# hfeeki/stellard

Hardware: AMD Instinct MI355X
Metric: Ed25519 tx verifies/sec (higher is better)
Workload: dtype u32

## Files before the change

### stellard_amd/build.py

```python
import os
import shutil
import subprocess
import sys

ROOT = os.path.dirname(os.path.dirname(os.path.abspath(__file__)))
CSRC = os.path.join(ROOT, "stellard_amd", "csrc")
HIPCC = shutil.which("hipcc") or "/opt/rocm/bin/hipcc"
ARCH = os.environ.get("PYTORCH_ROCM_ARCH", "gfx950")

PRODUCT_SRCS = ["stl_kernels.hip", "stl_keyset.hip", "stl_api.cpp", "stl_batcher.cpp"]
PRODUCT_DEPS = PRODUCT_SRCS + ["stl_kernels.h", "stl_verify_core.h", "stl_fe25519.h", "stl_ge25519.h",
                               "stl_sc25519.h", "stl_sha512.h", "stl_base_table.h", "stl_lattice.h", "stl_txblob.h", "stl_sign.h",
                               "stl_comb.h", "stl_keyset.h",
                               os.path.join("..", "..", "include", "stl.h")]


def source_digest():
    import hashlib
    h = hashlib.sha256()
    for d in PRODUCT_DEPS:
        with open(os.path.join(CSRC, d), "rb") as f:
            h.update(os.path.basename(d).encode() + b"\0" + f.read())
    return h.hexdigest()


def _stale(out, deps):
    if not os.path.exists(out):
        return True
    t = os.path.getmtime(out)
    return any(os.path.getmtime(d) > t for d in deps)


def _run(cmd, cwd=ROOT):
    print("+", " ".join(cmd), flush=True)
    subprocess.run(cmd, cwd=cwd, check=True)


HOST_DEPS = ["stl_kernels.h", "stl_keyset.h", os.path.join("..", "..", "include", "stl.h")]
OBJ_DIR = os.path.join(ROOT, "build", "obj")


def build_product(force=False, extra_flags=(), variant="variant"):
    out = os.path.join(ROOT, "stellard_amd", "libstl.so")
    deps = [os.path.join(CSRC, d) for d in PRODUCT_DEPS]
    if extra_flags:
        vout = os.path.join(ROOT, "build", "ab", variant + ".so")
        os.makedirs(os.path.dirname(vout), exist_ok=True)
        _run([HIPCC, f"--offload-arch={ARCH}", "-O3", "-std=c++17", "-fPIC", "-shared", *extra_flags,
              "-o", vout] + [os.path.join(CSRC, s) for s in PRODUCT_SRCS])
        return vout
    os.makedirs(OBJ_DIR, exist_ok=True)
    objs = []
    for src in PRODUCT_SRCS:
        obj = os.path.join(OBJ_DIR, src + ".o")
        if src.endswith(".hip"):
            sdeps = [d for d in deps if not d.endswith((".hip", ".cpp")) or d.endswith(src)]
        else:
            sdeps = [os.path.join(CSRC, d) for d in [src] + HOST_DEPS]
        if force or _stale(obj, sdeps):
            _run([HIPCC, f"--offload-arch={ARCH}", "-O3", "-std=c++17", "-fPIC", "-c", "-o", obj,
                  os.path.join(CSRC, src)])
        objs.append(obj)
    if force or _stale(out, objs):
        _run([HIPCC, f"--offload-arch={ARCH}", "-fPIC", "-shared", "-o", out] + objs)
    return out


def build_hostemu(force=False):
    out = os.path.join(ROOT, "tests", "native", "libhostemu.so")
    src = os.path.join(ROOT, "tests", "native", "hostemu.cpp")
    deps = [src] + [os.path.join(CSRC, d) for d in PRODUCT_DEPS]
    if force or _stale(out, deps):
        _run([HIPCC, "-O2", "-std=c++17", "-fPIC", "-shared", "-o", out, src])
    return out


def build_hostemu_keyset(force=False):
    out = os.path.join(ROOT, "tests", "native", "libhostemu_keyset.so")
    src = os.path.join(ROOT, "tests", "native", "hostemu_keyset.cpp")
    deps = [src] + [os.path.join(CSRC, d) for d in PRODUCT_DEPS]
    if force or _stale(out, deps):
        _run([HIPCC, "-O2", "-std=c++17", "-fPIC", "-shared", "-o", out, src])
    return out


def build_oracle():
    oracle = os.path.join(ROOT, "oracle")
    targets = ["build/liboracle.so"]
    if os.path.exists("/opt/conda/include/sodium.h"):
        targets.append("_ref/libsodium_ref.so")
    _run(["make", "-s", "-C", oracle] + targets)


def main(argv=None):
    argv = sys.argv[1:] if argv is None else argv
    force = "--force" in argv
    if "--product-only" in argv:
        build_product(force=force)
        return
    from concurrent.futures import ThreadPoolExecutor
    with ThreadPoolExecutor(max_workers=3) as ex:
        jobs = [ex.submit(build_product, force), ex.submit(build_hostemu, force),
                ex.submit(build_hostemu_keyset, force)]
        for j in jobs:
            j.result()
    build_oracle()


if __name__ == "__main__":
    main()
```

### stellard_amd/csrc/stl_api.cpp

```cpp
#include <dlfcn.h>
#include <hip/hip_runtime.h>
#include <rccl/rccl.h>

#include <algorithm>
#include <array>
#include <atomic>
#include <chrono>
#include <cstddef>
#include <cstdio>
#include <cstdlib>
#include <cstring>
#include <map>
#include <memory>
#include <mutex>
#include <set>
#include <thread>
#include <vector>

#include "../../include/stl.h"
#include "stl_kernels.h"
#include "stl_keyset.h"

namespace {

std::atomic<long long> g_fault_after{-1};

bool fault_now() {
  long long v = g_fault_after.load(std::memory_order_relaxed);
  while (v >= 0) {
    if (g_fault_after.compare_exchange_weak(v, v - 1, std::memory_order_relaxed)) return v == 0;
  }
  return false;
}

#define STL_TRY(expr)                        \
  do {                                       \
    if (fault_now()) return STL_EHIP;        \
    hipError_t e_ = (expr);                  \
    if (e_ != hipSuccess) return STL_EHIP;   \
  } while (0)

#define STL_RCCL_TRY(expr)                   \
  do {                                       \
    if (fault_now()) return STL_ERCCL;       \
    ncclResult_t r_ = (expr);                \
    if (r_ != ncclSuccess) return STL_ERCCL; \
  } while (0)

#define STL_RC(expr)        \
  do {                      \
    int rc_ = (expr);       \
    if (rc_) return rc_;    \
  } while (0)

struct Rccl {
  std::once_flag once;
  bool ok = false;
  decltype(&ncclGetUniqueId) GetUniqueId = nullptr;
  decltype(&ncclCommInitRank) CommInitRank = nullptr;
  decltype(&ncclCommInitAll) CommInitAll = nullptr;
  decltype(&ncclCommDestroy) CommDestroy = nullptr;
  decltype(&ncclGather) Gather = nullptr;
  decltype(&ncclAllGather) AllGather = nullptr;
  decltype(&ncclSend) Send = nullptr;
  decltype(&ncclRecv) Recv = nullptr;
  decltype(&ncclGroupStart) GroupStart = nullptr;
  decltype(&ncclGroupEnd) GroupEnd = nullptr;
  decltype(&ncclCommCount) CommCount = nullptr;
  decltype(&ncclCommUserRank) CommUserRank = nullptr;
  decltype(&ncclCommInitRankConfig) CommInitRankConfig = nullptr;
  decltype(&ncclCommGetAsyncError) CommGetAsyncError = nullptr;
  decltype(&ncclCommAbort) CommAbort = nullptr;
  bool nonblocking() const { return CommInitRankConfig && CommGetAsyncError && CommAbort; }

  template <typename F>
  static bool sym(void* h, const char* name, F& f) {
    f = reinterpret_cast<F>(dlsym(h, name));
    return f != nullptr;
  }
  bool load() {
    std::call_once(once, [this] {
      void* h = dlopen("librccl.so.1", RTLD_NOW | RTLD_GLOBAL);
      if (!h) h = dlopen("/opt/rocm/lib/librccl.so.1", RTLD_NOW | RTLD_GLOBAL);
      if (!h) return;
      ok = sym(h, "ncclGetUniqueId", GetUniqueId) && sym(h, "ncclCommInitRank", CommInitRank) &&
           sym(h, "ncclCommInitAll", CommInitAll) && sym(h, "ncclCommDestroy", CommDestroy) &&
           sym(h, "ncclGather", Gather) && sym(h, "ncclAllGather", AllGather) && sym(h, "ncclSend", Send) &&
           sym(h, "ncclRecv", Recv) && sym(h, "ncclGroupStart", GroupStart) && sym(h, "ncclGroupEnd", GroupEnd) &&
           sym(h, "ncclCommCount", CommCount) && sym(h, "ncclCommUserRank", CommUserRank);
      (void)(sym(h, "ncclCommInitRankConfig", CommInitRankConfig) &&
             sym(h, "ncclCommGetAsyncError", CommGetAsyncError) && sym(h, "ncclCommAbort", CommAbort));
    });
    return ok;
  }
};
Rccl g_rccl;

std::atomic<int> g_rccl_timeout_ms{120000};

int rccl_settle(ncclComm_t comm, ncclResult_t r) {
  if (r == ncclSuccess) return STL_OK;
  if (r != ncclInProgress || !comm || !g_rccl.CommGetAsyncError) return STL_ERCCL;
  const auto end = std::chrono::steady_clock::now() + std::chrono::milliseconds(g_rccl_timeout_ms.load());
  ncclResult_t st = ncclInProgress;
  while (g_rccl.CommGetAsyncError(comm, &st) == ncclSuccess && st == ncclInProgress) {
    if (std::chrono::steady_clock::now() > end) return STL_ERCCL;
    std::this_thread::sleep_for(std::chrono::microseconds(200));
  }
  return st == ncclSuccess ? STL_OK : STL_ERCCL;
}

struct DevBuf {
  void* p = nullptr;
  size_t cap = 0;
  int ensure(size_t bytes) {
    if (bytes <= cap) return STL_OK;
    if (p) (void)hipFree(p);
    p = nullptr;
    cap = 0;
    if (fault_now() || hipMalloc(&p, bytes) != hipSuccess) {
      p = nullptr;
      return STL_ENOMEM;
    }
    cap = bytes;
    return STL_OK;
  }
  void release() {
    if (p) (void)hipFree(p);
    p = nullptr;
    cap = 0;
  }
};

struct PhaseTimer {
  std::mutex mu;
  std::vector<hipEvent_t> pool;
  std::vector<std::array<hipEvent_t, 5>> done;
  uint64_t ns[4] = {0, 0, 0, 0};
  uint64_t chunks = 0;
  hipEvent_t take() {
    std::lock_guard<std::mutex> lk(mu);
    if (!pool.empty()) {
      hipEvent_t e = pool.back();
      pool.pop_back();
      return e;
    }
    hipEvent_t e = nullptr;
    if (hipEventCreate(&e) != hipSuccess) e = nullptr;
    return e;
  }
  void give(hipEvent_t e) {
    if (!e) return;
    std::lock_guard<std::mutex> lk(mu);
    pool.push_back(e);
  }
  void collect() {
    std::lock_guard<std::mutex> lk(mu);
    std::vector<std::array<hipEvent_t, 5>> pending;
    for (auto& c : done) {
      if (hipEventQuery(c[4]) == hipErrorNotReady) {
        pending.push_back(c);
        continue;
      }
      uint64_t t[4];
      bool ok = true;
      for (int i = 0; i < 4 && ok; ++i) {
        float ms = 0.f;
        ok = hipEventElapsedTime(&ms, c[i], c[i + 1]) == hipSuccess;
        t[i] = (uint64_t)((double)ms * 1e6);
      }
      if (ok) {
        for (int i = 0; i < 4; ++i) ns[i] += t[i];
        ++chunks;
      }
      for (hipEvent_t e : c) pool.push_back(e);
    }
    done.swap(pending);
  }
  void reset() {
    collect();
    std::lock_guard<std::mutex> lk(mu);
    for (auto& v : ns) v = 0;
    chunks = 0;
  }
  void release() {
    std::lock_guard<std::mutex> lk(mu);
    for (auto& c : done)
      for (hipEvent_t e : c) pool.push_back(e);
    done.clear();
    for (hipEvent_t e : pool) (void)hipEventDestroy(e);
    pool.clear();
  }
};

std::atomic<bool> g_phase_timing{false};

thread_local std::array<hipEvent_t, 5> t_marks;
thread_local bool t_marks_ok = false;

void phase_mark(void* ctx, hipStream_t s, int i) {
  auto* t = static_cast<PhaseTimer*>(ctx);
  if (i == 0) {
    for (hipEvent_t& m : t_marks) {
      if (m) (void)hipEventDestroy(m);
      m = nullptr;
    }
    t_marks_ok = true;
  }
  hipEvent_t e = t->take();
  if (!e || hipEventRecord(e, s) != hipSuccess) {
    t->give(e);
    t_marks[i] = nullptr;
    t_marks_ok = false;
  } else {
    t_marks[i] = e;
  }
  if (i == 4) {
    if (t_marks_ok) {
      std::lock_guard<std::mutex> lk(t->mu);
      t->done.push_back(t_marks);
    } else {
      for (hipEvent_t m : t_marks) t->give(m);
    }
    t_marks.fill(nullptr);
    t_marks_ok = false;
  }
}

std::atomic<int> g_tune_fused{1};
std::atomic<int> g_tune_queue{1};
std::atomic<int> g_tune_streams{2};
std::atomic<int> g_tune_sub_log2{0};
std::atomic<int> g_tune_byte_shards{0};
std::atomic<int> g_tune_quad{3};
std::atomic<int> g_tune_long_hash{8};
std::atomic<int> g_tune_shared_keys{1};
std::atomic<int> g_tune_wide_min{0};
std::atomic<int> g_tune_r_ahead{1};
std::atomic<int> g_tune_first_chunk{0};

std::atomic<uint64_t> g_shard_quantum{65536};

uint32_t pair_max_lanes(uint32_t grid);
uint32_t chunk_for(uint32_t grid, size_t n) {
  const int t = g_tune_sub_log2.load();
  if (t) return 1u << t;
  const size_t pm = pair_max_lanes(grid);
  if (n <= 2 * pm) return (uint32_t)std::min<size_t>(std::max<size_t>(n, 64), stl::kPreChunk);
  if (n <= 3 * pm) return (uint32_t)(2 * pm);
  const size_t nc = std::max<size_t>(2, (n + ((size_t)1 << 17)) >> 18);
  size_t sub = ((n + nc - 1) / nc + 63) / 64 * 64;
  sub = std::max<size_t>(sub, pair_max_lanes(grid) + 64);
  return (uint32_t)std::min<size_t>(sub, stl::kPreChunk);
}

struct StreamCtx;
struct CtxSpares {
  std::mutex mu;
  std::vector<std::unique_ptr<StreamCtx>> list;
};
std::atomic<int>& max_caller_streams();
struct StreamCtx {
  std::mutex mu;
  int ordinal = -1;
  bool pool = false;
  uint64_t last_use = 0;
  hipEvent_t done = nullptr;
  std::weak_ptr<CtxSpares> spares;
  DevBuf ws;
  DevBuf queue;
  hipEvent_t fork = nullptr;
  hipEvent_t join[stl::kMaxVerifyStreams] = {};
  hipEvent_t keys = nullptr;
  hipEvent_t parsed[2] = {};
  DevBuf rdec;
  hipEvent_t rready = nullptr;
  uint32_t* auto_flag = nullptr;
  uint32_t* auto_flag_dev = nullptr;
  DevBuf scratch;
  void release() {
    if (auto_flag) (void)hipHostFree(auto_flag);
    auto_flag = auto_flag_dev = nullptr;
    scratch.release();
    ws.release();
    queue.release();
    for (hipEvent_t& e : join) {
      if (e) (void)hipEventDestroy(e);
      e = nullptr;
    }
    if (fork) (void)hipEventDestroy(fork);
    fork = nullptr;
    if (keys) (void)hipEventDestroy(keys);
    keys = nullptr;
    for (hipEvent_t& e : parsed) {
      if (e) (void)hipEventDestroy(e);
      e = nullptr;
    }
    rdec.release();
    if (rready) (void)hipEventDestroy(rready);
    rready = nullptr;
    if (done) (void)hipEventDestroy(done);
    done = nullptr;
  }
  bool holds_memory() const {
    return auto_flag || scratch.p || ws.p || queue.p || fork || keys || parsed[0] || parsed[1] || rdec.p || rready ||
           done;
  }
  void adopt(StreamCtx& o) {
    std::swap(ws, o.ws);
    std::swap(queue, o.queue);
    std::swap(scratch, o.scratch);
    std::swap(fork, o.fork);
    std::swap(keys, o.keys);
    std::swap(parsed[0], o.parsed[0]);
    std::swap(parsed[1], o.parsed[1]);
    std::swap(rdec, o.rdec);
    std::swap(rready, o.rready);
    for (uint32_t j = 0; j < stl::kMaxVerifyStreams; ++j) std::swap(join[j], o.join[j]);
    std::swap(auto_flag, o.auto_flag);
    std::swap(auto_flag_dev, o.auto_flag_dev);
    std::swap(done, o.done);
  }
  ~StreamCtx() {
    if (!holds_memory() || ordinal < 0) return;
    if (done) {
      if (std::shared_ptr<CtxSpares> sp = spares.lock()) {
        auto z = std::make_unique<StreamCtx>();
        z->ordinal = ordinal;
        z->adopt(*this);
        std::unique_ptr<StreamCtx> over;
        {
          std::lock_guard<std::mutex> lk(sp->mu);
          sp->list.push_back(std::move(z));
          if (sp->list.size() > (size_t)max_caller_streams().load()) {
            over = std::move(sp->list.front());
            sp->list.erase(sp->list.begin());
          }
        }
        return;
      }
    }
    int prev = -1;
    (void)hipGetDevice(&prev);
    if (hipSetDevice(ordinal) == hipSuccess) (void)hipDeviceSynchronize();
    release();
    if (prev >= 0) (void)hipSetDevice(prev);
  }
};

std::unique_ptr<StreamCtx> take_spare(CtxSpares& sp) {
  std::lock_guard<std::mutex> lk(sp.mu);
  if (sp.list.empty()) return nullptr;
  size_t pick = 0;
  for (size_t i = 0; i < sp.list.size(); ++i)
    if (sp.list[i]->done && hipEventQuery(sp.list[i]->done) == hipSuccess) {
      pick = i;
      break;
    }
  std::unique_ptr<StreamCtx> z = std::move(sp.list[pick]);
  sp.list.erase(sp.list.begin() + (long)pick);
  return z;
}

struct Device {
  int ordinal = 0;
  int cus = 0;
  uint32_t grid = 0;
  hipStream_t stream = nullptr;
  hipStream_t stream2 = nullptr;
  hipStream_t copy = nullptr;
  std::atomic<hipStream_t> stream3{nullptr};
  ncclComm_t comm = nullptr;
  std::mutex mu;
  DevBuf sig, msg, pk, bitmap, pre, off, len, ctr, ctr2, txid, status, wide, gather;
  DevBuf counters;
  std::map<hipStream_t, std::shared_ptr<StreamCtx>> stream_ws;
  std::shared_ptr<CtxSpares> spares = std::make_shared<CtxSpares>();
  uint64_t ws_tick = 0;
  std::mutex ws_mu;
  void* stage = nullptr;
  size_t stage_cap = 0;
  PhaseTimer timer;
  stl::PhaseClock clock{phase_mark, &timer};
};

const stl::PhaseClock* phase_clock(Device& d) { return g_phase_timing.load() ? &d.clock : nullptr; }

std::mutex g_mu;
std::vector<std::unique_ptr<Device>> g_devs;
bool g_init = false;
int g_shards_per_device = 1;
bool g_comm_gather = false;
std::atomic<stl_verify_fn> g_fallback_verify{nullptr};

std::mutex g_pcomm_mu;
ncclComm_t g_pcomm = nullptr;
int g_pcomm_ranks = 0;
hipEvent_t g_gather_start = nullptr;
hipStream_t g_gather_stream = nullptr;

void pcomm_abort_locked() {
  if (g_pcomm && g_rccl.ok) (void)(g_rccl.CommAbort ? g_rccl.CommAbort(g_pcomm) : g_rccl.CommDestroy(g_pcomm));
  g_pcomm = nullptr;
  g_pcomm_ranks = 0;
}

void mark_gather_start(hipStream_t s) {
  if (!g_gather_start && hipEventCreateWithFlags(&g_gather_start, hipEventDisableTiming) != hipSuccess) {
    g_gather_start = nullptr;
    g_gather_stream = nullptr;
    return;
  }
  g_gather_stream = hipEventRecord(g_gather_start, s) == hipSuccess ? s : nullptr;
}

unsigned long long* dev_counters(Device& d) { return static_cast<unsigned long long*>(d.counters.p); }

std::atomic<uint64_t> g_st_batches{0}, g_st_sigs{0}, g_st_errors{0}, g_st_host_ns{0}, g_st_gather_ns{0},
    g_st_auto_dedup{0};
bool g_trace = false;

uint64_t now_ns() {
  return (uint64_t)std::chrono::duration_cast<std::chrono::nanoseconds>(
             std::chrono::steady_clock::now().time_since_epoch())
      .count();
}

struct CallSpan {
  const char* name;
  size_t n;
  uint64_t t0 = now_ns();
  int finish(int rc, uint64_t gather_ns = 0) {
    const uint64_t dt = now_ns() - t0;
    g_st_batches++;
    g_st_sigs += n;
    g_st_host_ns += dt;
    g_st_gather_ns += gather_ns;
    if (rc < 0) g_st_errors++;
    if (g_trace)
      std::fprintf(stderr, "{\"stl_trace\": \"%s\", \"n\": %zu, \"rc\": %d, \"ms\": %.3f, \"gather_ms\": %.3f}\n", name, n,
                   rc, dt * 1e-6, gather_ns * 1e-6);
    return rc;
  }
};

struct DeviceGuard {
  int prev = -1;
  DeviceGuard() {
    if (hipGetDevice(&prev) != hipSuccess) prev = -1;
  }
  ~DeviceGuard() {
    if (prev >= 0) (void)hipSetDevice(prev);
  }
};

int current_device_index() {
  int ord = -1;
  if (hipGetDevice(&ord) != hipSuccess) return -1;
  for (size_t i = 0; i < g_devs.size(); ++i)
    if (g_devs[i]->ordinal == ord) return (int)i;
  return -1;
}

int setup_device(Device& d) {
  STL_TRY(hipSetDevice(d.ordinal));
  hipDeviceProp_t prop;
  STL_TRY(hipGetDeviceProperties(&prop, d.ordinal));
  if (std::strncmp(prop.gcnArchName, "gfx950", 6) != 0) return STL_ENODEV;
  d.cus = prop.multiProcessorCount;
  int per_cu = 0;
  STL_TRY(hipOccupancyMaxActiveBlocksPerMultiprocessor(&per_cu, stl::kernel_verify_msg32(), stl::kBlock, 0));
  if (per_cu < 1) per_cu = 1;
  d.grid = (uint32_t)(d.cus * per_cu);
  g_shard_quantum.store((uint64_t)d.grid * stl::kBlock / 2);
  STL_TRY(hipStreamCreateWithFlags(&d.stream, hipStreamNonBlocking));
  STL_TRY(hipStreamCreateWithFlags(&d.stream2, hipStreamNonBlocking));
  STL_TRY(hipStreamCreateWithFlags(&d.copy, hipStreamNonBlocking));
  STL_RC(d.counters.ensure(64));
  STL_TRY(hipMemsetAsync(d.counters.p, 0, 64, d.stream));
  STL_RC(d.wide.ensure(stl::kWideTableBytes));
  STL_TRY(stl::launch_wide_table(static_cast<uint4*>(d.wide.p), d.stream));
  STL_TRY(hipStreamSynchronize(d.stream));
  return STL_OK;
}

void release_device(Device& d) {
  (void)hipSetDevice(d.ordinal);
  const hipStream_t s3 = d.stream3.load();
  for (hipStream_t s : {d.stream, d.stream2, s3, d.copy})
    if (s) (void)hipStreamSynchronize(s);
  (void)hipDeviceSynchronize();
  if (d.comm && g_rccl.ok) (void)g_rccl.CommDestroy(d.comm);
  d.comm = nullptr;
  for (DevBuf* b : {&d.sig, &d.msg, &d.pk, &d.bitmap, &d.pre, &d.off, &d.len, &d.ctr, &d.ctr2, &d.txid, &d.status,
                    &d.wide, &d.gather, &d.counters})
    b->release();
  {
    std::lock_guard<std::mutex> lk(d.ws_mu);
    for (auto& kv : d.stream_ws) {
      std::lock_guard<std::mutex> cl(kv.second->mu);
      kv.second->release();
    }
    d.stream_ws.clear();
    if (std::shared_ptr<CtxSpares> sp = std::move(d.spares)) {
      std::lock_guard<std::mutex> sl(sp->mu);
      for (auto& z : sp->list) z->release();
      sp->list.clear();
    }
  }
  if (d.stage) (void)hipHostFree(d.stage);
  d.stage = nullptr;
  d.stage_cap = 0;
  d.timer.release();
  for (hipStream_t s : {d.stream, d.stream2, s3, d.copy})
    if (s) (void)hipStreamDestroy(s);
  d.stream = d.stream2 = d.copy = nullptr;
  d.stream3.store(nullptr);
}

int ensure_init() {
  {
    std::lock_guard<std::mutex> lk(g_mu);
    if (g_init) return STL_OK;
  }
  return stl_init(nullptr);
}

constexpr int kDefaultCallerStreams = 8;
std::atomic<int> g_max_caller_streams{kDefaultCallerStreams};
std::atomic<int>& max_caller_streams() { return g_max_caller_streams; }

bool is_pool_stream(const Device& d, hipStream_t s) {
  return s && (s == d.stream || s == d.stream2 || s == d.copy || s == d.stream3.load());
}

struct CtxUse {
  std::shared_ptr<StreamCtx> c;
  hipStream_t s = nullptr;
  ~CtxUse() {
    if (!c || c->pool || !c->done) return;
    std::lock_guard<std::mutex> lk(c->mu);
    (void)hipEventRecord(c->done, s);
  }
};

std::shared_ptr<StreamCtx> stream_ctx(Device& d, hipStream_t s) {
  std::vector<std::shared_ptr<StreamCtx>> evicted;
  std::shared_ptr<StreamCtx> out;
  {
    std::lock_guard<std::mutex> lk(d.ws_mu);
    auto& slot = d.stream_ws[s];
    if (!slot) {
      slot = std::make_shared<StreamCtx>();
      slot->ordinal = d.ordinal;
      slot->pool = is_pool_stream(d, s);
      if (!slot->pool) {
        std::vector<std::pair<uint64_t, hipStream_t>> callers;
        for (auto& kv : d.stream_ws)
          if (!kv.second->pool && kv.first != s) callers.emplace_back(kv.second->last_use, kv.first);
        std::sort(callers.begin(), callers.end());
        const size_t keep = (size_t)std::max(0, g_max_caller_streams.load() - 1);
        for (size_t i = 0; i + keep < callers.size(); ++i) {
          auto it = d.stream_ws.find(callers[i].second);
          evicted.push_back(std::move(it->second));
          d.stream_ws.erase(it);
        }
      }
      if (!slot->pool && d.spares) {
        slot->spares = d.spares;
        StreamCtx* src = nullptr;
        for (auto& e : evicted)
          if (!src && e.use_count() == 1 && e->done) src = e.get();
        std::unique_ptr<StreamCtx> z;
        if (!src && (z = take_spare(*d.spares))) src = z.get();
        if (src) {
          slot->adopt(*src);
          if (slot->done && hipStreamWaitEvent(s, slot->done, 0) != hipSuccess) (void)hipEventSynchronize(slot->done);
        }
        if (!slot->done && hipEventCreateWithFlags(&slot->done, hipEventDisableTiming) != hipSuccess)
          slot->done = nullptr;
      }
    }
    out = d.stream_ws[s];
    out->last_use = ++d.ws_tick;
  }
  if (out->pool) return out;
  auto use = std::make_shared<CtxUse>();
  use->c = out;
  use->s = s;
  return std::shared_ptr<StreamCtx>(use, use->c.get());
}

int caller_contexts(Device& d) {
  std::lock_guard<std::mutex> lk(d.ws_mu);
  int k = 0;
  for (auto& kv : d.stream_ws) k += kv.second->pool ? 0 : 1;
  return k;
}

uint32_t verify_grid_for(const Device& d, size_t n) {
  const size_t tiles = (n + stl::kBlock - 1) / stl::kBlock;
  return (uint32_t)std::max<size_t>(1, std::min<size_t>(2 * tiles, d.grid));
}

uint32_t pair_max_lanes(uint32_t grid) { return grid * stl::kBlock / 4; }
uint32_t pair_max(const Device& d) { return pair_max_lanes(d.grid); }
uint32_t quad_max(const Device& d) { return (g_tune_quad.load() & 1) ? d.grid * stl::kBlock / 16 : 0u; }
uint32_t duo_max(const Device& d) { return (g_tune_quad.load() & 2) ? d.grid * stl::kBlock / 8 : 0u; }

unsigned long long* dev_counters(Device& d);
const stl::PhaseClock* phase_clock(Device& d);

hipStream_t key_stream_for(const Device& d, const hipStream_t* used, uint32_t S) {
  for (hipStream_t c : {d.stream, d.stream2}) {
    bool taken = c == nullptr;
    for (uint32_t j = 0; j < S; ++j) taken = taken || used[j] == c;
    if (!taken) return c;
  }
  return nullptr;
}

int run_verify(Device& d, hipStream_t s, const uint8_t* sig, const uint8_t* msg_or_k, const uint8_t* pk, size_t n,
               uint64_t* words, uint32_t mode, bool pre_k, int streams, bool concurrent = false) {
  const bool dedup = (mode & stl::kModeDedupKeys) != 0;
  stl::VerifyExec x;
  x.grid = verify_grid_for(d, n);
  x.ws_grid = d.grid;
  x.pair_max = pair_max(d);
  x.quad_max = quad_max(d);
  x.duo_max = duo_max(d);
  x.wide = static_cast<const uint4*>(d.wide.p);
  x.counters = dev_counters(d);
  x.clock = phase_clock(d);
  x.fused_prep = g_tune_fused.load();
  x.main_queue = g_tune_queue.load() != 0;
  x.concurrent = concurrent;
  x.sub = chunk_for(d.grid, n);
  x.first = (uint32_t)g_tune_first_chunk.load();
  uint32_t S = (uint32_t)std::max(1, std::min<int>(streams, (int)stl::kMaxVerifyStreams));
  if (x.clock || n <= x.sub || x.sub <= x.pair_max) S = 1;
  S = (uint32_t)std::min<size_t>(S, (n + x.sub - 1) / x.sub);
  hipStream_t pool[stl::kMaxVerifyStreams] = {s};
  uint32_t np = 1;
  if (S > 1) {
    if (S > 3 && !d.stream3.load()) {
      std::lock_guard<std::mutex> lk(d.ws_mu);
      if (!d.stream3.load()) {
        hipStream_t s3 = nullptr;
        STL_TRY(hipStreamCreateWithFlags(&s3, hipStreamNonBlocking));
        d.stream3.store(s3);
      }
    }
    for (hipStream_t p : {d.stream2, d.stream, d.stream3.load()})
      if (np < S && p && p != s) pool[np++] = p;
  }
  S = np;
  x.nstreams = S;
  std::shared_ptr<StreamCtx> hold[stl::kMaxVerifyStreams];
  StreamCtx* ctx[stl::kMaxVerifyStreams];
  for (uint32_t j = 0; j < S; ++j) {
    hold[j] = stream_ctx(d, pool[j]);
    ctx[j] = hold[j].get();
  }
  StreamCtx* order[stl::kMaxVerifyStreams];
  std::copy(ctx, ctx + S, order);
  std::sort(order, order + S);
  std::vector<std::unique_lock<std::mutex>> locks;
  for (uint32_t j = 0; j < S; ++j) locks.emplace_back(order[j]->mu);
  StreamCtx& c = *ctx[0];
  for (uint32_t j = 0; j < S; ++j) {
    STL_RC(ctx[j]->ws.ensure(stl::verify_ws_bytes(d.grid, dedup)));
    x.ws[j] = static_cast<uint4*>(ctx[j]->ws.p);
    x.streams[j] = pool[j];
    if (j > 0) {
      if (!c.join[j]) STL_TRY(hipEventCreateWithFlags(&c.join[j], hipEventDisableTiming));
      x.join[j] = c.join[j];
    }
  }
  if (S > 1 && !c.fork) STL_TRY(hipEventCreateWithFlags(&c.fork, hipEventDisableTiming));
  x.fork = c.fork;
  x.wide_min = (uint32_t)g_tune_wide_min.load();
  if (S > 1 && dedup && g_tune_shared_keys.load()) {
    if (!c.keys) STL_TRY(hipEventCreateWithFlags(&c.keys, hipEventDisableTiming));
    x.key_ready = c.keys;
    x.key_stream = key_stream_for(d, pool, S);
  }
  if (fault_now() || stl::launch_verify(sig, msg_or_k, pk, (uint32_t)n, words, mode, pre_k, x) != hipSuccess) {
    for (uint32_t j = 1; j < S; ++j) (void)hipStreamSynchronize(pool[j]);
    if (x.key_stream) (void)hipStreamSynchronize(x.key_stream);
    return STL_EHIP;
  }
  return STL_OK;
}

int ctx_queue(StreamCtx& c, size_t n, uint32_t** qws, bool blob = false) {
  STL_RC(c.queue.ensure(blob ? stl::blob_queue_bytes(n) : stl::hash_queue_bytes(n)));
  *qws = static_cast<uint32_t*>(c.queue.p);
  return STL_OK;
}

uint32_t hash_grid(const Device& d) { return (uint32_t)d.cus * 8u; }

uint32_t hash_long_min(const Device& d, size_t n) {
  return n <= 2 * (size_t)pair_max(d) ? (uint32_t)g_tune_long_hash.load() : 0u;
}

uint32_t grid_for(const Device& d, size_t n) {
  const size_t tiles = (n + stl::kBlock - 1) / stl::kBlock;
  return (uint32_t)std::max<size_t>(1, std::min<size_t>(tiles, d.grid));
}

void shard(size_t n, int r, int g, size_t* lo, size_t* hi) {
  const size_t words = (n + 63) / 64;
  const size_t per = (words + g - 1) / g;
  *lo = std::min(n, (size_t)r * per * 64);
  *hi = std::min(n, (size_t)(r + 1) * per * 64);
}


void shard_bytes_bounds(const uint32_t* len, size_t n, int g, std::vector<size_t>& bound) {
  bound.assign(g + 1, n);
  bound[0] = 0;
  uint64_t total = 0;
  for (size_t i = 0; i < n; ++i) total += len[i];
  const uint64_t q = g_shard_quantum.load();
  uint64_t acc = 0;
  size_t i = 0;
  for (int r = 1; r < g; ++r) {
    const uint64_t target = (uint64_t)((__uint128_t)total * (unsigned)r / (unsigned)g);
    while (i < n && acc < target) acc += len[i++];
    size_t b = std::min(n, (i + 63) / 64 * 64);
    if (q >= 64 && q % 64 == 0 && n > q) {
      auto prefix = [&](size_t row) {
        uint64_t p = acc;
        if (row >= i)
          for (size_t k = i; k < row; ++k) p += len[k];
        else
          for (size_t k = row; k < i; ++k) p -= len[k];
        return p;
      };
      const size_t down = b / q * q, up = down + q;
      const size_t c = (b - down <= up - b || up > n) ? down : up;
      const uint64_t pc = prefix(c);
      const uint64_t dev = pc > target ? pc - target : target - pc;
      if (c > 0 && c < n && (__uint128_t)dev * (unsigned)g * 40u <= (__uint128_t)total) b = c;
    }
    bound[r] = std::max(bound[r - 1], b);
  }
}

#ifndef STL_PIPE_CHUNK_LOG2
#define STL_PIPE_CHUNK_LOG2 16
#endif
constexpr size_t kPipeChunk = (size_t)1 << STL_PIPE_CHUNK_LOG2;

enum class Mode { kSig, kPre, kBlob };

struct Batch {
  Mode mode;
  const uint8_t *sig, *msg32, *pk, *bytes;
  const uint64_t* off;
  const uint32_t* len;
  uint8_t *bitmap, *status, *txid;
  uint32_t policy, kind;
  bool auto_dedup;
};

const uint8_t* row_key(const Batch& b, size_t i) {
  if (b.mode != Mode::kBlob) return b.pk + 32 * i;
  const uint8_t* p = b.bytes + b.off[i];
  const size_t len = b.len[i], lim = len < 34 ? 0 : std::min<size_t>(len - 34, 256);
  for (size_t j = 0; j + 1 <= lim; ++j)
    if (p[j] == 0x73 && p[j + 1] == 0x20) return p + j + 2;
  return nullptr;
}

bool keys_repeat(const Batch& b, size_t lo, size_t hi) {
  constexpr size_t kSample = 1024, kSlots = 2048;
  const size_t n = hi - lo;
  if (n < 4 * 64) return false;
  const size_t s = std::min(n, kSample);
  uint64_t table[kSlots] = {};
  size_t dups = 0;
  for (size_t k = 0; k < s; ++k) {
    const uint8_t* key = row_key(b, lo + k * n / s);
    if (!key) continue;
    uint64_t a, c;
    std::memcpy(&a, key, 8);
    std::memcpy(&c, key + 24, 8);
    uint64_t f = (a ^ (c * 0x9E3779B97F4A7C15ull)) | 1u;
    size_t h = (size_t)((f * 0xD6E8FEB86659FD93ull) >> 52) & (kSlots - 1);
    while (table[h] && table[h] != f) h = (h + 1) & (kSlots - 1);
    if (table[h] == f) ++dups;
    table[h] = f;
  }
  return 5 * dups >= s;
}

uint32_t chunk_policy(const Batch& b, size_t lo, size_t hi) {
  if (!b.auto_dedup || !keys_repeat(b, lo, hi)) return b.policy;
  g_st_auto_dedup++;
  return b.policy | stl::kModeDedupKeys;
}

struct Shard {
  Device* d = nullptr;
  size_t lo = 0, hi = 0;
  std::vector<uint64_t> roff, row_end;
  std::vector<hipEvent_t> ev;
  int rc = STL_OK;
  ~Shard() {
    for (hipEvent_t e : ev) (void)hipEventDestroy(e);
  }
  int join(hipStream_t from, hipStream_t to) {
    hipEvent_t e;
    STL_TRY(hipEventCreateWithFlags(&e, hipEventDisableTiming));
    ev.push_back(e);
    STL_TRY(hipEventRecord(e, from));
    STL_TRY(hipStreamWaitEvent(to, e, 0));
    return STL_OK;
  }
};

void rebase(const uint64_t* off, const uint32_t* len, size_t lo, size_t hi, std::vector<uint64_t>& roff,
            std::vector<uint64_t>& row_end, uint64_t* base_out, uint64_t* bytes_out) {
  const size_t n = hi - lo;
  uint64_t base = off[lo], end = 0;
  for (size_t i = lo; i < hi; ++i) base = std::min(base, off[i]);
  roff.resize(n);
  row_end.resize(n);
  for (size_t i = 0; i < n; ++i) {
    roff[i] = off[lo + i] - base;
    row_end[i] = roff[i] + len[lo + i];
    end = std::max(end, row_end[i]);
  }
  *base_out = base;
  *bytes_out = end;
}

int copy_rows(Shard& s, uint8_t* dst, const uint8_t* src, size_t c0, size_t c1, uint64_t* watermark) {
  uint64_t need = *watermark;
  for (size_t i = c0; i < c1; ++i) need = std::max(need, s.row_end[i]);
  if (need > *watermark)
    STL_TRY(hipMemcpyAsync(dst + *watermark, src + *watermark, need - *watermark, hipMemcpyHostToDevice, s.d->copy));
  *watermark = need;
  return STL_OK;
}

int enqueue_shard(const Batch& b, Shard& s, size_t words_alloc) {
  Device& d = *s.d;
  const size_t lo = s.lo, n = s.hi - s.lo;
  STL_TRY(hipSetDevice(d.ordinal));
  STL_RC(d.bitmap.ensure(std::max<size_t>(words_alloc, 1) * 8));
  if (n == 0) return STL_OK;
  STL_RC(d.sig.ensure(n * 64));
  STL_RC(d.msg.ensure(n * 32));
  STL_RC(d.pk.ensure(n * 32));
  uint64_t base = 0, bytes = 0, mark = 0;
  uint8_t* dsig = static_cast<uint8_t*>(d.sig.p);
  uint8_t* dmsg = static_cast<uint8_t*>(d.msg.p);
  uint8_t* dpk = static_cast<uint8_t*>(d.pk.p);
  uint8_t* dpre = nullptr;
  uint64_t* doff = nullptr;
  uint32_t* dlen = nullptr;
  if (b.mode != Mode::kSig) {
    rebase(b.off, b.len, lo, s.hi, s.roff, s.row_end, &base, &bytes);
    STL_RC(d.pre.ensure(bytes + 16));
    STL_RC(d.off.ensure(n * 8));
    STL_RC(d.len.ensure(n * 4));
    const size_t qn = std::min(n, kPipeChunk);
    const size_t qbytes = b.mode == Mode::kBlob ? stl::blob_queue_bytes(qn) : stl::hash_queue_bytes(qn);
    STL_RC(d.ctr.ensure(qbytes));
    if (b.mode == Mode::kBlob) {
      STL_RC(d.status.ensure(n));
      if (b.txid) STL_RC(d.txid.ensure(n * 32));
    }
    dpre = static_cast<uint8_t*>(d.pre.p);
    doff = static_cast<uint64_t*>(d.off.p);
    dlen = static_cast<uint32_t*>(d.len.p);
    STL_TRY(hipMemcpyAsync(doff, s.roff.data(), n * 8, hipMemcpyHostToDevice, d.copy));
    STL_TRY(hipMemcpyAsync(dlen, b.len + lo, n * 4, hipMemcpyHostToDevice, d.copy));
  }
  uint8_t* dtxid = (b.mode == Mode::kBlob && b.txid) ? static_cast<uint8_t*>(d.txid.p) : nullptr;
  uint8_t* dstatus = b.mode == Mode::kBlob ? static_cast<uint8_t*>(d.status.p) : nullptr;
  const bool two = g_tune_streams.load() > 1 && n > kPipeChunk && !phase_clock(d);
  if (b.auto_dedup && n > kPipeChunk / 2)
    for (hipStream_t ks : {d.stream, d.stream2}) {
      const std::shared_ptr<StreamCtx> c = stream_ctx(d, ks);
      std::lock_guard<std::mutex> lk(c->mu);
      STL_RC(c->ws.ensure(stl::verify_ws_bytes(d.grid, true)));
    }
  if (two && b.mode != Mode::kSig) {
    const size_t qn = std::min(n, kPipeChunk);
    STL_RC(d.ctr2.ensure(b.mode == Mode::kBlob ? stl::blob_queue_bytes(qn) : stl::hash_queue_bytes(qn)));
  }
  for (size_t c0 = 0; c0 < n; c0 += kPipeChunk) {
    const size_t c1 = std::min(n, c0 + kPipeChunk), cn = c1 - c0;
    const bool odd = two && ((c0 / kPipeChunk) & 1);
    hipStream_t ks = odd ? d.stream2 : d.stream;
    uint32_t* kctr = static_cast<uint32_t*>((odd ? d.ctr2 : d.ctr).p);
    if (b.mode != Mode::kBlob) {
      STL_TRY(hipMemcpyAsync(dsig + 64 * c0, b.sig + 64 * (lo + c0), cn * 64, hipMemcpyHostToDevice, d.copy));
      STL_TRY(hipMemcpyAsync(dpk + 32 * c0, b.pk + 32 * (lo + c0), cn * 32, hipMemcpyHostToDevice, d.copy));
    }
    if (b.mode == Mode::kSig)
      STL_TRY(hipMemcpyAsync(dmsg + 32 * c0, b.msg32 + 32 * (lo + c0), cn * 32, hipMemcpyHostToDevice, d.copy));
    else
      STL_RC(copy_rows(s, dpre, b.bytes + base, c0, c1, &mark));
    STL_RC(s.join(d.copy, ks));
    if (b.mode == Mode::kPre)
      STL_TRY(stl::launch_tx_hash(dpre, doff + c0, dlen + c0, (uint32_t)cn, dmsg + 32 * c0, kctr, hash_grid(d), ks,
                                  hash_long_min(d, n)));
    else if (b.mode == Mode::kBlob)
      STL_TRY(stl::launch_tx_blob(dpre, doff + c0, dlen + c0, (uint32_t)cn, dmsg + 32 * c0, dsig + 64 * c0,
                                  dpk + 32 * c0, dtxid ? dtxid + 32 * c0 : nullptr, dstatus + c0, kctr,
                                  hash_grid(d), ks, b.kind));
    STL_RC(run_verify(d, ks, dsig + 64 * c0, dmsg + 32 * c0, dpk + 32 * c0, cn,
                      static_cast<uint64_t*>(d.bitmap.p) + c0 / 64, chunk_policy(b, lo + c0, lo + c1), false, 1,
                      two));
  }
  if (two) STL_RC(s.join(d.stream2, d.stream));
  if (dstatus && b.status) STL_TRY(hipMemcpyAsync(b.status + lo, dstatus, n, hipMemcpyDeviceToHost, d.stream));
  if (dtxid) STL_TRY(hipMemcpyAsync(b.txid + 32 * lo, dtxid, n * 32, hipMemcpyDeviceToHost, d.stream));
  return STL_OK;
}

int drain(Device& d) {
  (void)hipSetDevice(d.ordinal);
  const hipError_t a = hipStreamSynchronize(d.copy);
  const hipError_t b = hipStreamSynchronize(d.stream);
  const hipError_t c = hipStreamSynchronize(d.stream2);
  const hipStream_t s3 = d.stream3.load();
  const hipError_t e = s3 ? hipStreamSynchronize(s3) : hipSuccess;
  return (a == hipSuccess && b == hipSuccess && c == hipSuccess && e == hipSuccess) ? STL_OK : STL_EHIP;
}

int finish_direct(const Batch& b, Shard& s, std::vector<uint8_t>& host_words) {
  const size_t n = s.hi - s.lo;
  if (n == 0) return STL_OK;
  host_words.resize((n + 63) / 64 * 8);
  STL_TRY(hipMemcpyAsync(host_words.data(), s.d->bitmap.p, host_words.size(), hipMemcpyDeviceToHost, s.d->stream));
  STL_TRY(hipStreamSynchronize(s.d->stream));
  std::memcpy(b.bitmap + s.lo / 8, host_words.data(), (n + 7) / 8);
  return STL_OK;
}

int run_shard_direct(const Batch& b, Shard& s) {
  std::lock_guard<std::mutex> lk(s.d->mu);
  int rc = enqueue_shard(b, s, (s.hi - s.lo + 63) / 64);
  std::vector<uint8_t> host_words;
  if (rc == STL_OK) rc = finish_direct(b, s, host_words);
  const int drc = drain(*s.d);
  return rc ? rc : drc;
}

int gather_to_host(const Batch& b, std::vector<Shard>& sh, size_t n, size_t per, bool equal) {
  const int g = (int)sh.size();
  Device& root = *sh[0].d;
  const size_t words = (n + 63) / 64;
  STL_TRY(hipSetDevice(root.ordinal));
  STL_RC(root.gather.ensure(std::max(words, per * (size_t)g) * 8));
  uint64_t* rbuf = static_cast<uint64_t*>(root.gather.p);
  STL_RCCL_TRY(g_rccl.GroupStart());
  int rc = STL_OK;
  for (int r = 0; r < g; ++r) {
    Device& d = *sh[r].d;
    const uint64_t* sbuf = static_cast<const uint64_t*>(d.bitmap.p);
    if (equal) {
      if (g_rccl.Gather(sbuf, rbuf, per, ncclUint64, 0, d.comm, d.stream) != ncclSuccess) rc = STL_ERCCL;
    } else {
      const size_t w = (sh[r].hi - sh[r].lo + 63) / 64;
      if (w == 0 || r == 0) continue;
      const bool sent = g_rccl.Send(sbuf, w, ncclUint64, 0, d.comm, d.stream) == ncclSuccess;
      const bool recv = g_rccl.Recv(rbuf + sh[r].lo / 64, w, ncclUint64, r, root.comm, root.stream) == ncclSuccess;
      if (!sent || !recv) rc = STL_ERCCL;
    }
  }
  if (g_rccl.GroupEnd() != ncclSuccess && rc == STL_OK) rc = STL_ERCCL;
  if (rc) return rc;
  STL_TRY(hipSetDevice(root.ordinal));
  if (!equal && sh[0].hi > sh[0].lo)
    STL_TRY(hipMemcpyAsync(rbuf, root.bitmap.p, (sh[0].hi - sh[0].lo + 63) / 64 * 8, hipMemcpyDeviceToDevice,
                           root.stream));
  std::vector<uint8_t> host_words(words * 8);
  STL_TRY(hipMemcpyAsync(host_words.data(), rbuf, words * 8, hipMemcpyDeviceToHost, root.stream));
  STL_TRY(hipStreamSynchronize(root.stream));
  std::memcpy(b.bitmap, host_words.data(), (n + 7) / 8);
  return STL_OK;
}

int check_flags(uint32_t flags) {
  return (flags & ~(STL_POLICY_MASK | STL_REQUIRE_S_LT_L | STL_FULL_LENGTH | STL_DEDUP_KEYS | STL_ONE_LANE |
                    STL_NO_AUTO_DEDUP | STL_DEBUG_RAW_PREDICATE))
             ? STL_EINVAL
             : STL_OK;
}

bool auto_dedup(uint32_t flags) {
  return (flags & (STL_DEDUP_KEYS | STL_NO_AUTO_DEDUP | STL_FULL_LENGTH)) == 0;
}

constexpr size_t kSmallBatch = 4096;

int run_small(const Batch& b, size_t n) {
  Device& d = *g_devs[0];
  std::lock_guard<std::mutex> lk(d.mu);
  STL_TRY(hipSetDevice(d.ordinal));
  const size_t bytes = n * 128, words = (n + 63) / 64;
  if (d.stage_cap < bytes + words * 8) {
    if (d.stage) (void)hipHostFree(d.stage);
    d.stage = nullptr;
    d.stage_cap = 0;
    const size_t cap = kSmallBatch * 128 + kSmallBatch / 8;
    if (fault_now() || hipHostMalloc(&d.stage, cap, hipHostMallocDefault) != hipSuccess) {
      d.stage = nullptr;
      return STL_ENOMEM;
    }
    d.stage_cap = cap;
  }
  STL_RC(d.sig.ensure(bytes));
  STL_RC(d.bitmap.ensure(words * 8));
  uint8_t* st = static_cast<uint8_t*>(d.stage);
  std::memcpy(st, b.sig, n * 64);
  std::memcpy(st + 64 * n, b.msg32, n * 32);
  std::memcpy(st + 96 * n, b.pk, n * 32);
  uint8_t* dev = static_cast<uint8_t*>(d.sig.p);
  auto go = [&]() -> int {
    STL_TRY(hipMemcpyAsync(dev, st, bytes, hipMemcpyHostToDevice, d.stream));
    STL_RC(run_verify(d, d.stream, dev, dev + 64 * n, dev + 96 * n, n, static_cast<uint64_t*>(d.bitmap.p),
                      chunk_policy(b, 0, n), false, 1));
    STL_TRY(hipMemcpyAsync(st + bytes, d.bitmap.p, words * 8, hipMemcpyDeviceToHost, d.stream));
    STL_TRY(hipStreamSynchronize(d.stream));
    return STL_OK;
  };
  const int rc = go();
  if (rc) {
    (void)hipStreamSynchronize(d.stream);
    return rc;
  }
  std::memcpy(b.bitmap, st + bytes, (n + 7) / 8);
  return STL_OK;
}

int run_batch(const Batch& b, size_t n, uint64_t* gather_ns) {
  if (n == 0) return STL_OK;
  STL_RC(ensure_init());
  DeviceGuard guard;
  const int g = (int)g_devs.size();
  if (g == 0) return STL_ENODEV;
  if (b.mode == Mode::kSig && n <= kSmallBatch && g == 1 && g_shards_per_device == 1 && !g_comm_gather)
    return run_small(b, n);
  const size_t kMaxShard = (size_t)1 << 31;
  int gg = g * g_shards_per_device;
  while ((n + gg - 1) / gg > kMaxShard) gg += g;
  std::vector<size_t> bound;
  const bool by_bytes = b.mode != Mode::kSig && (gg > 1 || g_tune_byte_shards.load() != 0);
  if (by_bytes) shard_bytes_bounds(b.len, n, gg, bound);
  std::vector<Shard> sh(gg);
  for (int r = 0; r < gg; ++r) {
    sh[r].d = g_devs[r % g].get();
    if (by_bytes) {
      sh[r].lo = bound[r];
      sh[r].hi = bound[r + 1];
    } else {
      shard(n, r, gg, &sh[r].lo, &sh[r].hi);
    }
  }
  if (g_comm_gather && gg == g) {
    std::vector<std::unique_lock<std::mutex>> locks;
    for (auto& d : g_devs) locks.emplace_back(d->mu);
    size_t per = 1;
    for (auto& s : sh) per = std::max(per, (s.hi - s.lo + 63) / 64);
    std::vector<std::thread> th;
    for (int r = 0; r < gg; ++r) {
      if (r + 1 == gg) sh[r].rc = enqueue_shard(b, sh[r], per);
      else th.emplace_back([&, r] { sh[r].rc = enqueue_shard(b, sh[r], per); });
    }
    for (auto& t : th) t.join();
    int rc = STL_OK;
    for (auto& s : sh) rc = rc ? rc : s.rc;
    if (rc == STL_OK) {
      const uint64_t g0 = now_ns();
      rc = gather_to_host(b, sh, n, per, !by_bytes);
      *gather_ns = now_ns() - g0;
    }
    for (auto& d : g_devs) {
      const int drc = drain(*d);
      rc = rc ? rc : drc;
    }
    return rc;
  }
  std::vector<std::thread> th;
  for (int r = 0; r < gg; ++r) {
    if (r + 1 == gg) sh[r].rc = run_shard_direct(b, sh[r]);
    else th.emplace_back([&, r] { sh[r].rc = run_shard_direct(b, sh[r]); });
  }
  for (auto& t : th) t.join();
  for (auto& s : sh)
    if (s.rc) return s.rc;
  return STL_OK;
}

int env_int(const char* name, int dflt) {
  const char* v = std::getenv(name);
  return (v && *v) ? std::atoi(v) : dflt;
}

}

struct stl_keyset {
  int ordinal = -1;
  uint32_t nkeys = 0;
  std::vector<uint8_t> pk;
  std::map<std::array<uint8_t, 32>, uint32_t> first;
  DevBuf rec, tables;
  size_t table_bytes() const { return ((size_t)nkeys + 1) * stl::keyset_key_words() * 4; }
  const uint32_t* d_rec() const { return static_cast<const uint32_t*>(rec.p); }
  const uint32_t* d_tables() const { return static_cast<const uint32_t*>(tables.p); }
};

namespace {
std::mutex g_ks_mu;
std::set<const stl_keyset*> g_keysets;

void keyset_free_locked(stl_keyset* ks) {
  g_keysets.erase(ks);
  DeviceGuard guard;
  if (hipSetDevice(ks->ordinal) == hipSuccess) (void)hipDeviceSynchronize();
  ks->rec.release();
  ks->tables.release();
  delete ks;
}

void keysets_release_all() {
  std::lock_guard<std::mutex> lk(g_ks_mu);
  while (!g_keysets.empty()) keyset_free_locked(const_cast<stl_keyset*>(*g_keysets.begin()));
}

int check_keyset_flags(uint32_t flags) {
  return (flags & ~(STL_POLICY_MASK | STL_REQUIRE_S_LT_L | STL_DEBUG_RAW_PREDICATE)) ? STL_EINVAL : STL_OK;
}
}

extern "C" {

int stl_init(const stl_config* cfg) {
  std::lock_guard<std::mutex> lk(g_mu);
  if (!g_init) {
    const char* fa = std::getenv("STL_FAULT_AFTER");
    if (fa && *fa) g_fault_after.store(std::atoll(fa));
    g_trace = env_int("STL_TRACE", 0) != 0;
    if (env_int("STL_PHASE_TIMING", 0) != 0) g_phase_timing.store(true);
    const int s = env_int("STL_STREAMS", 0), c = env_int("STL_CHUNK_LOG2", 0);
    if (s >= 1 && s <= (int)stl::kMaxVerifyStreams) g_tune_streams.store(s);
    const int to = env_int("STL_RCCL_TIMEOUT_S", 0);
    if (to > 0 && to <= 3600) g_rccl_timeout_ms.store(to * 1000);
    const int ws = env_int("STL_MAX_STREAM_WORKSPACES", 0);
    if (ws >= 1 && ws <= 64) g_max_caller_streams.store(ws);
    if (c >= 15 && c <= 20) g_tune_sub_log2.store(c);
  }
  int first = 0, want = -1, spd = 1;
  uint32_t cflags = 0;
  if (cfg) {
    const uint32_t abi1 = 4 * sizeof(uint32_t), abi2 = offsetof(stl_config, fallback_verify);
    const uint32_t sz = cfg->struct_size;
    if (sz != sizeof(stl_config) && sz != abi1 && sz != abi2) return STL_EINVAL;
    first = cfg->first_device;
    if (cfg->device_count > 0) want = cfg->device_count;
    cflags = cfg->flags;
    if ((cflags & ~(STL_CFG_RCCL_GATHER | STL_CFG_NO_RCCL)) ||
        (cflags & (STL_CFG_RCCL_GATHER | STL_CFG_NO_RCCL)) == (STL_CFG_RCCL_GATHER | STL_CFG_NO_RCCL) ||
        first < 0)
      return STL_EINVAL;
    if (sz >= abi2) {
      if (cfg->reserved != 0) return STL_EINVAL;
      if (cfg->shards_per_device > 0) spd = cfg->shards_per_device;
    }
    if (sz == sizeof(stl_config)) g_fallback_verify.store(cfg->fallback_verify);
  }
  int count = 0;
  if (hipGetDeviceCount(&count) != hipSuccess || count <= 0) return g_init ? STL_OK : STL_ENODEV;
  if (want < 0) want = count;
  if (std::getenv("STL_DEVICES")) want = std::max(1, env_int("STL_DEVICES", want));
  spd = std::max(1, std::min(64, env_int("STL_SHARDS_PER_DEVICE", spd)));
  const int env_rccl = env_int("STL_RCCL", -1);
  if (env_rccl == 1) cflags = (cflags & ~STL_CFG_NO_RCCL) | STL_CFG_RCCL_GATHER;
  if (env_rccl == 0) cflags = (cflags & ~STL_CFG_RCCL_GATHER) | STL_CFG_NO_RCCL;
  if (first < 0 || first >= count) return STL_EINVAL;
  want = std::min(want, count - first);
  const bool gather = !(cflags & STL_CFG_NO_RCCL) && spd == 1 && (cflags & STL_CFG_RCCL_GATHER);
  if (g_init) {
    if (!cfg) return STL_OK;
    const bool same = !g_devs.empty() && g_devs[0]->ordinal == first && (int)g_devs.size() == want &&
                      gather == g_comm_gather && spd == g_shards_per_device;
    return same ? STL_OK : STL_EINVAL;
  }
  int prev = 0;
  (void)hipGetDevice(&prev);
  auto fail = [&](int rc) {
    for (auto& d : g_devs) release_device(*d);
    g_devs.clear();
    (void)hipSetDevice(prev);
    return rc;
  };
  for (int i = 0; i < want; ++i) {
    std::unique_ptr<Device> d(new Device());
    d->ordinal = first + i;
    g_devs.push_back(std::move(d));
    const int rc = setup_device(*g_devs.back());
    if (rc) return fail(rc);
  }
  if (gather) {
    if (!g_rccl.load() || fault_now()) return fail(STL_ERCCL);
    std::vector<ncclComm_t> comms(want);
    std::vector<int> ords(want);
    for (int i = 0; i < want; ++i) ords[i] = g_devs[i]->ordinal;
    if (g_rccl.CommInitAll(comms.data(), want, ords.data()) != ncclSuccess) return fail(STL_ERCCL);
    for (int i = 0; i < want; ++i) g_devs[i]->comm = comms[i];
  }
  (void)hipSetDevice(prev);
  g_shards_per_device = spd;
  g_comm_gather = gather;
  g_init = true;
  return STL_OK;
}

void stl_shutdown(void) {
  stl_comm_destroy();
  keysets_release_all();
  DeviceGuard guard;
  std::lock_guard<std::mutex> lk(g_mu);
  for (auto& d : g_devs) {
    std::lock_guard<std::mutex> dl(d->mu);
    release_device(*d);
  }
  g_devs.clear();
  g_comm_gather = false;
  g_shards_per_device = 1;
  g_init = false;
}

int stl_device_count(void) {
  std::lock_guard<std::mutex> lk(g_mu);
  return (int)g_devs.size();
}

const char* stl_version(void) { return "stl 0.3.0 (gfx950, abi 4)"; }

const char* stl_strerror(int rc) {
  switch (rc) {
    case STL_OK: return "ok";
    case STL_EINVAL: return "invalid argument";
    case STL_ENODEV: return "no gfx950 device";
    case STL_ENOMEM: return "out of memory";
    case STL_EHIP: return "HIP runtime error";
    case STL_ERCCL: return "RCCL error";
    default: return "unknown error";
  }
}

void stl_debug_fault_after(long long calls) { g_fault_after.store(calls < 0 ? -1 : calls); }

int stl_debug_tuning(int key, int value) {
  if (value == -1) {
    switch (key) {
      case STL_TUNE_FUSED_PREP: return g_tune_fused.load();
      case STL_TUNE_MAIN_QUEUE: return g_tune_queue.load();
      case STL_TUNE_STREAMS: return g_tune_streams.load();
      case STL_TUNE_CHUNK_LOG2: return g_tune_sub_log2.load();
      case STL_TUNE_BYTE_SHARDS: return g_tune_byte_shards.load();
      case STL_TUNE_QUAD: return g_tune_quad.load();
      case STL_TUNE_STREAM_WORKSPACES: return g_max_caller_streams.load();
      case STL_TUNE_RCCL_TIMEOUT_MS: return g_rccl_timeout_ms.load();
      case STL_TUNE_LONG_HASH: return g_tune_long_hash.load();
      default: return STL_EINVAL;
    }
  }
  switch (key) {
    case STL_TUNE_FUSED_PREP:
      if (value < 0 || value > 1) return STL_EINVAL;
      return g_tune_fused.exchange(value);
    case STL_TUNE_MAIN_QUEUE:
      if (value != 0 && value != 1) return STL_EINVAL;
      return g_tune_queue.exchange(value);
    case STL_TUNE_STREAMS:
      if (value < 1 || value > (int)stl::kMaxVerifyStreams) return STL_EINVAL;
      return g_tune_streams.exchange(value);
    case STL_TUNE_CHUNK_LOG2:
      if (value != 0 && (value < 15 || value > 20)) return STL_EINVAL;
      return g_tune_sub_log2.exchange(value);
    case STL_TUNE_BYTE_SHARDS:
      if (value != 0 && value != 1) return STL_EINVAL;
      return g_tune_byte_shards.exchange(value);
    case STL_TUNE_QUAD:
      if (value < 0 || value > 3) return STL_EINVAL;
      return g_tune_quad.exchange(value);
    case STL_TUNE_STREAM_WORKSPACES:
      if (value < 1 || value > 64) return STL_EINVAL;
      return g_max_caller_streams.exchange(value);
    case STL_TUNE_RCCL_TIMEOUT_MS:
      if (value < 1 || value > 3600000) return STL_EINVAL;
      return g_rccl_timeout_ms.exchange(value);
    case STL_TUNE_LONG_HASH:
      if (value < 0 || value > 62) return STL_EINVAL;
      return g_tune_long_hash.exchange(value);
    case STL_TUNE_SHARED_KEYS:
      if (value != 0 && value != 1) return STL_EINVAL;
      return g_tune_shared_keys.exchange(value);
    case STL_TUNE_FIRST_CHUNK:
      if (value < 0 || value % 64 != 0 || value > (1 << 20)) return STL_EINVAL;
      return g_tune_first_chunk.exchange(value);
    case STL_TUNE_R_AHEAD:
      if (value != 0 && value != 1) return STL_EINVAL;
      return g_tune_r_ahead.exchange(value);
    case STL_TUNE_WIDE_MIN_ROWS:
      if (value < 0 || value > (int)stl::kPreChunk) return STL_EINVAL;
      return g_tune_wide_min.exchange(value);
    default:
      return STL_EINVAL;
  }
}

int stl_release_stream(void* stream) {
  const hipStream_t s = static_cast<hipStream_t>(stream);
  std::shared_ptr<StreamCtx> gone;
  {
    std::lock_guard<std::mutex> lk(g_mu);
    if (!g_init) return STL_OK;
    const int di = current_device_index();
    if (di < 0) return STL_ENODEV;
    Device& d = *g_devs[di];
    if (is_pool_stream(d, s)) return STL_EINVAL;
    std::lock_guard<std::mutex> wl(d.ws_mu);
    auto it = d.stream_ws.find(s);
    if (it == d.stream_ws.end()) return STL_OK;
    gone = std::move(it->second);
    d.stream_ws.erase(it);
  }
  return STL_OK;
}

int stl_debug_stream_contexts(void) {
  std::lock_guard<std::mutex> lk(g_mu);
  if (!g_init) return 0;
  const int di = current_device_index();
  return di < 0 ? STL_ENODEV : caller_contexts(*g_devs[di]);
}

int stl_get_stats(stl_stats* out) {
  if (!out || (out->struct_size != sizeof(stl_stats) && out->struct_size != offsetof(stl_stats, auto_dedup_chunks)))
    return STL_EINVAL;
  if (out->struct_size == sizeof(stl_stats)) out->auto_dedup_chunks = g_st_auto_dedup.load();
  out->batches = g_st_batches.load();
  out->signatures = g_st_sigs.load();
  out->errors = g_st_errors.load();
  out->host_ns = g_st_host_ns.load();
  out->gather_ns = g_st_gather_ns.load();
  out->accepted = 0;
  out->full_length_lanes = 0;
  for (auto& v : out->phase_ns) v = 0;
  out->phase_chunks = 0;
  DeviceGuard guard;
  std::lock_guard<std::mutex> lk(g_mu);
  for (auto& d : g_devs) {
    if (!d->counters.p) continue;
    unsigned long long c[2] = {0, 0};
    if (hipSetDevice(d->ordinal) != hipSuccess || hipDeviceSynchronize() != hipSuccess ||
        hipMemcpy(c, d->counters.p, sizeof c, hipMemcpyDeviceToHost) != hipSuccess)
      return STL_EHIP;
    out->accepted += c[0];
    out->full_length_lanes += c[1];
    d->timer.collect();
    std::lock_guard<std::mutex> tl(d->timer.mu);
    for (int i = 0; i < 4; ++i) out->phase_ns[i] += d->timer.ns[i];
    out->phase_chunks += d->timer.chunks;
  }
  return STL_OK;
}

void stl_reset_stats(void) {
  g_st_batches = 0;
  g_st_sigs = 0;
  g_st_errors = 0;
  g_st_host_ns = 0;
  g_st_gather_ns = 0;
  g_st_auto_dedup = 0;
  DeviceGuard guard;
  std::lock_guard<std::mutex> lk(g_mu);
  for (auto& d : g_devs)
    if (d->counters.p && hipSetDevice(d->ordinal) == hipSuccess) {
      (void)hipMemset(d->counters.p, 0, 64);
      (void)hipDeviceSynchronize();
      d->timer.reset();
    }
}

int stl_set_phase_timing(int on) { return g_phase_timing.exchange(on != 0) ? 1 : 0; }

void stl_shard_range(size_t n, int r, int g, size_t* lo, size_t* hi) {
  if (!lo || !hi) return;
  if (g < 1 || r < 0 || r >= g) {
    *lo = *hi = n;
    return;
  }
  shard(n, r, g, lo, hi);
}

void stl_shard_range_bytes(const uint32_t* len, size_t n, int r, int g, size_t* lo, size_t* hi) {
  if (!lo || !hi) return;
  if (g < 1 || r < 0 || r >= g || (n && !len)) {
    *lo = *hi = n;
    return;
  }
  std::vector<size_t> bound;
  shard_bytes_bounds(len, n, g, bound);
  *lo = bound[r];
  *hi = bound[r + 1];
}

int stl_ed25519_verify_batch(const uint8_t* sig, const uint8_t* msg, const uint8_t* pk, size_t n,
                             uint8_t* accept_bitmap, uint32_t flags) {
  if (n == 0) return STL_OK;
  if (!sig || !msg || !pk || !accept_bitmap) return STL_EINVAL;
  STL_RC(check_flags(flags));
  const Batch b{Mode::kSig, sig, msg, pk, nullptr, nullptr, nullptr, accept_bitmap, nullptr, nullptr,
                stl::kernel_mode(flags), 0u, auto_dedup(flags)};
  CallSpan span{"stl_ed25519_verify_batch", n};
  uint64_t g = 0;
  const int rc = run_batch(b, n, &g);
  return span.finish(rc, g);
}

int stl_tx_verify_batch(const uint8_t* preimages, const uint64_t* offset, const uint32_t* len, const uint8_t* sig,
                        const uint8_t* pk, size_t n, uint8_t* accept_bitmap, uint32_t flags) {
  if (n == 0) return STL_OK;
  if (!preimages || !offset || !len || !sig || !pk || !accept_bitmap) return STL_EINVAL;
  STL_RC(check_flags(flags));
  const Batch b{Mode::kPre, sig, nullptr, pk, preimages, offset, len, accept_bitmap, nullptr, nullptr,
                stl::kernel_mode(flags), 0u, auto_dedup(flags)};
  CallSpan span{"stl_tx_verify_batch", n};
  uint64_t g = 0;
  const int rc = run_batch(b, n, &g);
  return span.finish(rc, g);
}

int stl_signed_blob_verify_batch(uint32_t kind, const uint8_t* blobs, const uint64_t* offset, const uint32_t* len,
                                 size_t n, uint8_t* accept_bitmap, uint8_t* status, uint8_t* id, uint32_t flags) {
  if (kind != STL_BLOB_TRANSACTION && kind != STL_BLOB_VALIDATION) return STL_EINVAL;
  if (n == 0) return STL_OK;
  if (!blobs || !offset || !len || !accept_bitmap) return STL_EINVAL;
  STL_RC(check_flags(flags));
  const Batch b{Mode::kBlob, nullptr, nullptr, nullptr, blobs, offset, len, accept_bitmap, status, id,
                stl::kernel_mode(flags), kind, auto_dedup(flags)};
  CallSpan span{kind == STL_BLOB_VALIDATION ? "stl_signed_blob_verify_batch(validation)" : "stl_tx_blob_verify_batch",
                n};
  uint64_t g = 0;
  const int rc = run_batch(b, n, &g);
  return span.finish(rc, g);
}

int stl_tx_blob_verify_batch(const uint8_t* blobs, const uint64_t* offset, const uint32_t* len, size_t n,
                             uint8_t* accept_bitmap, uint8_t* status, uint8_t* tx_id, uint32_t flags) {
  return stl_signed_blob_verify_batch(STL_BLOB_TRANSACTION, blobs, offset, len, n, accept_bitmap, status, tx_id,
                                      flags);
}

namespace {
int verify_detached_device(const uint8_t* sig, const uint8_t* m, unsigned long long mlen, const uint8_t* pk);
bool s_lt_l(const uint8_t* S);
}

int stl_ed25519_verify_detached(const uint8_t* sig, const uint8_t* m, unsigned long long mlen, const uint8_t* pk) {
  if (!sig || !pk || (mlen && !m)) return STL_EINVAL;
  const stl_verify_fn fb = g_fallback_verify.load();
  const int rc = mlen > 0xffffffffull ? STL_EINVAL : verify_detached_device(sig, m, mlen, pk);
  if (rc >= -1 || fb == nullptr) return rc;
  return (fb(sig, m, mlen, pk) == 0 && s_lt_l(sig + 32)) ? 0 : -1;
}

namespace {
bool s_lt_l(const uint8_t* S) {
  static const uint8_t L[32] = {0xed, 0xd3, 0xf5, 0x5c, 0x1a, 0x63, 0x12, 0x58, 0xd6, 0x9c, 0xf7,
                                0xa2, 0xde, 0xf9, 0xde, 0x14, 0x00, 0x00, 0x00, 0x00, 0x00, 0x00,
                                0x00, 0x00, 0x00, 0x00, 0x00, 0x00, 0x00, 0x00, 0x00, 0x10};
  for (int i = 31; i >= 0; --i)
    if (S[i] != L[i]) return S[i] < L[i];
  return false;
}

int verify_detached_device(const uint8_t* sig, const uint8_t* m, unsigned long long mlen, const uint8_t* pk) {
  if (mlen == 32) {
    uint8_t bit = 0;
    const int rc = stl_ed25519_verify_batch(sig, m, pk, 1, &bit, STL_POLICY_SODIUM_1_0_18);
    if (rc) return rc;
    return (bit & 1) ? 0 : -1;
  }
  if (mlen > 0xffffffffull) return STL_EINVAL;
  STL_RC(ensure_init());
  DeviceGuard guard;
  Device& d = *g_devs[0];
  std::lock_guard<std::mutex> lk(d.mu);
  STL_TRY(hipSetDevice(d.ordinal));
  STL_RC(d.sig.ensure(64));
  STL_RC(d.pk.ensure(32));
  STL_RC(d.msg.ensure(32));
  STL_RC(d.bitmap.ensure(8));
  STL_RC(d.pre.ensure(mlen ? mlen : 1));
  STL_RC(d.off.ensure(16));
  hipStream_t s = d.stream;
  const uint64_t hostmeta[2] = {0, mlen};
  uint64_t word = 0;
  auto enqueue = [&]() -> int {
    STL_TRY(hipMemcpyAsync(d.sig.p, sig, 64, hipMemcpyHostToDevice, s));
    STL_TRY(hipMemcpyAsync(d.pk.p, pk, 32, hipMemcpyHostToDevice, s));
    if (mlen) STL_TRY(hipMemcpyAsync(d.pre.p, m, mlen, hipMemcpyHostToDevice, s));
    STL_TRY(hipMemcpyAsync(d.off.p, hostmeta, 16, hipMemcpyHostToDevice, s));
    uint64_t* meta = static_cast<uint64_t*>(d.off.p);
    STL_TRY(stl::launch_hram_var(static_cast<uint8_t*>(d.sig.p), static_cast<uint8_t*>(d.pk.p),
                                 static_cast<uint8_t*>(d.pre.p), meta, meta + 1, 1, static_cast<uint8_t*>(d.msg.p), s));
    STL_RC(run_verify(d, s, static_cast<uint8_t*>(d.sig.p), static_cast<uint8_t*>(d.msg.p),
                      static_cast<uint8_t*>(d.pk.p), 1, static_cast<uint64_t*>(d.bitmap.p), STL_POLICY_SODIUM_1_0_18,
                      true, 1));
    STL_TRY(hipMemcpyAsync(&word, d.bitmap.p, 8, hipMemcpyDeviceToHost, s));
    STL_TRY(hipStreamSynchronize(s));
    return STL_OK;
  };
  const int rc = enqueue();
  const int drc = drain(d);
  if (rc || drc) return rc ? rc : drc;
  return (word & 1) ? 0 : -1;
}
}

namespace {
int device_for_call(Device** out) {
  STL_RC(ensure_init());
  const int di = current_device_index();
  if (di < 0) return STL_ENODEV;
  *out = g_devs[di].get();
  return STL_OK;
}
}

namespace {
int auto_dedup_device(StreamCtx& c, uint32_t flags, uint32_t* mode, uint32_t** flag_dev) {
  *flag_dev = nullptr;
  if (!auto_dedup(flags)) return STL_OK;
  std::lock_guard<std::mutex> lk(c.mu);
  if (!c.auto_flag) {
    void* p = nullptr;
    STL_TRY(hipHostMalloc(&p, 64, hipHostMallocMapped | hipHostMallocCoherent));
    c.auto_flag = static_cast<uint32_t*>(p);
    *c.auto_flag = 0;
    void* dp = nullptr;
    if (hipHostGetDevicePointer(&dp, p, 0) != hipSuccess) {
      (void)hipHostFree(p);
      c.auto_flag = nullptr;
      return STL_EHIP;
    }
    c.auto_flag_dev = static_cast<uint32_t*>(dp);
  }
  if (__atomic_load_n(c.auto_flag, __ATOMIC_ACQUIRE) == 1u) {
    *mode |= stl::kModeDedupKeys;
    g_st_auto_dedup++;
  }
  *flag_dev = c.auto_flag_dev;
  return STL_OK;
}
}

namespace {
int checksign_device(Device& d, hipStream_t s, bool blob, uint32_t kind, const uint8_t* bytes, const uint64_t* off,
                     const uint32_t* len, const uint8_t* sig_in, const uint8_t* pk_in, size_t n, uint64_t* words,
                     uint8_t* status, uint8_t* id, uint32_t flags) {
  const stl::PhaseClock* clock = phase_clock(d);
  size_t sub = chunk_for(d.grid, n);
  uint32_t S = (uint32_t)std::max(1, std::min(g_tune_streams.load(), 2));
  if (clock || n <= sub) {
    S = 1;
    sub = std::min<size_t>(n, stl::kPreChunk);
  }
  hipStream_t ks[2] = {s, s == d.stream2 ? d.stream : d.stream2};
  const std::shared_ptr<StreamCtx> hold[2] = {stream_ctx(d, ks[0]),
                                              S > 1 ? stream_ctx(d, ks[1]) : std::shared_ptr<StreamCtx>()};
  StreamCtx* kc[2] = {hold[0].get(), hold[1].get()};
  StreamCtx& c = *kc[0];
  uint32_t mode = stl::kernel_mode(flags);
  uint32_t* flag_dev = nullptr;
  STL_RC(auto_dedup_device(c, flags, &mode, &flag_dev));
  const bool dedup = (mode & stl::kModeDedupKeys) != 0;
  auto exec_for = [&](uint32_t cnt, uint32_t j) {
    stl::VerifyExec x;
    x.grid = verify_grid_for(d, cnt);
    x.ws_grid = d.grid;
    x.pair_max = pair_max(d);
    x.quad_max = quad_max(d);
    x.duo_max = duo_max(d);
    x.wide = static_cast<const uint4*>(d.wide.p);
    x.counters = dev_counters(d);
    x.clock = S > 1 ? nullptr : clock;
    x.fused_prep = g_tune_fused.load();
    x.main_queue = g_tune_queue.load() != 0;
    x.concurrent = S > 1;
    x.nstreams = 1;
    x.streams[0] = ks[j];
    x.ws[0] = static_cast<uint4*>(kc[j]->ws.p);
    return x;
  };
  const bool ahead = S == 1 && !blob && !clock && n <= stl::kPreChunk &&
                     stl::verify_pair_points((uint32_t)n, mode, exec_for((uint32_t)n, 0));
  std::vector<std::unique_lock<std::mutex>> locks;
  if (S > 1 && kc[1] < kc[0]) locks.emplace_back(kc[1]->mu);
  locks.emplace_back(c.mu);
  if (S > 1 && kc[1] > kc[0]) locks.emplace_back(kc[1]->mu);
  uint32_t* q[2] = {nullptr, nullptr};
  STL_RC(ctx_queue(*kc[0], S > 1 ? sub : n, &q[0], blob));
  if (S > 1) STL_RC(ctx_queue(*kc[1], n - sub, &q[1], blob));
  const size_t row = blob ? 128 : 32;
  STL_RC(c.scratch.ensure(std::max<size_t>(n, 1) * row));
  uint8_t* msg = static_cast<uint8_t*>(c.scratch.p);
  uint8_t* sig = blob ? msg + 32 * n : const_cast<uint8_t*>(sig_in);
  uint8_t* pk = blob ? msg + 96 * n : const_cast<uint8_t*>(pk_in);
  uint8_t* st = status;
  for (uint32_t j = 0; j < S; ++j) STL_RC(kc[j]->ws.ensure(stl::verify_ws_bytes(d.grid, dedup)));
  const bool shared_keys = dedup && S > 1 && n <= stl::kPreChunk && sub > pair_max(d) && g_tune_shared_keys.load();
  hipStream_t cs = shared_keys ? key_stream_for(d, ks, S) : nullptr;
  if (shared_keys && !c.keys) STL_TRY(hipEventCreateWithFlags(&c.keys, hipEventDisableTiming));
  if (cs && blob)
    for (hipEvent_t& e : c.parsed)
      if (!e) STL_TRY(hipEventCreateWithFlags(&e, hipEventDisableTiming));
  hipStream_t cr = cs && g_tune_r_ahead.load() && d.copy != cs && d.copy != ks[0] && d.copy != ks[1] ? d.copy
                                                                                                      : nullptr;
  if (cr) {
    STL_RC(c.rdec.ensure(n * 80));
    if (!c.rready) STL_TRY(hipEventCreateWithFlags(&c.rready, hipEventDisableTiming));
  }
  if (S > 1 || ahead) {
    if (!c.fork) STL_TRY(hipEventCreateWithFlags(&c.fork, hipEventDisableTiming));
    if (!c.join[1]) STL_TRY(hipEventCreateWithFlags(&c.join[1], hipEventDisableTiming));
    if (!c.join[2]) STL_TRY(hipEventCreateWithFlags(&c.join[2], hipEventDisableTiming));
    STL_TRY(hipEventRecord(c.fork, s));
    STL_TRY(hipStreamWaitEvent(ks[1], c.fork, 0));
  }
  auto fail = [&](int rc) {
    if (S > 1 || ahead) (void)hipStreamSynchronize(ks[1]);
    if (cs) (void)hipStreamSynchronize(cs);
    if (cr) (void)hipStreamSynchronize(cr);
    return rc;
  };
  if (ahead) {
    int rc = STL_OK;
    if (fault_now() || stl::launch_verify_points(sig, pk, (uint32_t)n, mode, exec_for((uint32_t)n, 0), ks[1]) !=
                           hipSuccess)
      rc = STL_EHIP;
    if (!rc && flag_dev && stl::launch_key_sample(pk, (uint32_t)n, flag_dev, ks[1]) != hipSuccess) rc = STL_EHIP;
    if (!rc && hipEventRecord(c.join[2], ks[1]) != hipSuccess) rc = STL_EHIP;
    if (rc) return fail(rc);
  }
  const bool split_pass = blob && cs && S > 1;
  auto parse = [&](size_t b0, size_t cnt, hipStream_t js, uint32_t* qw) -> int {
    if (fault_now()) return STL_EHIP;
    const hipError_t e = stl::launch_tx_blob_parse(bytes, off + b0, len + b0, (uint32_t)cnt, msg + 32 * b0,
                                                   sig + 64 * b0, pk + 32 * b0, id ? id + 32 * b0 : nullptr, st + b0,
                                                   qw, hash_grid(d), js, kind, c.parsed[js == ks[0] ? 0 : 1]);
    return e == hipSuccess ? STL_OK : STL_EHIP;
  };
  auto hash = [&](size_t b0, size_t cnt, hipStream_t js, uint32_t* qw) -> int {
    hipError_t e;
    if (split_pass) {
      e = stl::launch_tx_blob_hash(bytes, off + b0, len + b0, (uint32_t)cnt, msg + 32 * b0, sig + 64 * b0,
                                   pk + 32 * b0, id ? id + 32 * b0 : nullptr, st + b0, qw, hash_grid(d), js, kind);
      return e == hipSuccess ? STL_OK : STL_EHIP;
    }
    if (fault_now()) return STL_EHIP;
    if (blob)
      e = stl::launch_tx_blob(bytes, off + b0, len + b0, (uint32_t)cnt, msg + 32 * b0, sig + 64 * b0, pk + 32 * b0,
                              id ? id + 32 * b0 : nullptr, st + b0, qw, hash_grid(d), js, kind,
                              cs ? c.parsed[js == ks[0] ? 0 : 1] : nullptr);
    else
      e = stl::launch_tx_hash(bytes, off + b0, len + b0, (uint32_t)cnt, msg + 32 * b0, qw, hash_grid(d), js,
                              hash_long_min(d, n));
    return e == hipSuccess ? STL_OK : STL_EHIP;
  };
  auto hash_all = [&]() -> int {
    if (S == 1) {
      int rc = hash(0, n, s, q[0]);
      if (!rc && ahead && hipStreamWaitEvent(s, c.join[2], 0) != hipSuccess) rc = STL_EHIP;
      return rc;
    }
    int rc = hash(0, sub, ks[0], q[0]);
    if (!rc) rc = hash(sub, n - sub, ks[1], q[1]);
    if (!rc && hipEventRecord(c.join[2], ks[1]) != hipSuccess) rc = STL_EHIP;
    return rc;
  };
  if (split_pass) {
    int rc = parse(0, sub, ks[0], q[0]);
    if (!rc) rc = parse(sub, n - sub, ks[1], q[1]);
    if (rc) return fail(rc);
  } else if (int rc = hash_all()) {
    return fail(rc);
  }
  if (cs) {
    hipError_t e = hipSuccess;
    if (blob) {
      e = hipStreamWaitEvent(cs, c.parsed[0], 0);
      if (e == hipSuccess) e = hipStreamWaitEvent(cs, c.parsed[1], 0);
    } else {
      e = hipStreamWaitEvent(cs, c.fork, 0);
    }
    if (e == hipSuccess && fault_now()) e = hipErrorUnknown;
    if (e == hipSuccess)
      e = stl::launch_key_domain_ws(pk, (uint32_t)n, static_cast<uint4*>(kc[0]->ws.p), d.grid,
                                    (uint32_t)g_tune_wide_min.load(), cs);
    if (e == hipSuccess) e = hipEventRecord(c.keys, cs);
    if (e != hipSuccess) return fail(STL_EHIP);
  }
  if (cr) {
    hipError_t e = hipSuccess;
    if (blob) {
      e = hipStreamWaitEvent(cr, c.parsed[0], 0);
      if (e == hipSuccess) e = hipStreamWaitEvent(cr, c.parsed[1], 0);
    } else {
      e = hipStreamWaitEvent(cr, c.fork, 0);
    }
    if (e == hipSuccess && fault_now()) e = hipErrorUnknown;
    const size_t last = n - (n - 1) / sub * sub;
    const bool last_pairs = n > sub && !(mode & stl::kModeOneLane) && last <= pair_max(d);
    const size_t r_rows = last_pairs ? n - last : n;
    if (e == hipSuccess)
      e = stl::launch_point_r(sig, pk, (uint32_t)r_rows, mode, static_cast<uint4*>(c.rdec.p), cr);
    if (e == hipSuccess) e = hipEventRecord(c.rready, cr);
    if (e != hipSuccess) return fail(STL_EHIP);
  }
  if (split_pass)
    if (int rc = hash_all()) return fail(rc);
  size_t k = 0;
  for (size_t b0 = 0; b0 < n; b0 += sub, ++k) {
    const uint32_t j = (uint32_t)(k % S);
    const uint32_t cnt = (uint32_t)std::min(sub, n - b0);
    hipStream_t js = ks[j];
    if (S > 1 && k == 2 && hipStreamWaitEvent(ks[0], c.join[2], 0) != hipSuccess) return fail(STL_EHIP);
    stl::VerifyExec x = exec_for(cnt, j);
    x.points_done = ahead;
    if (shared_keys) {
      x.key_ws = static_cast<uint4*>(kc[0]->ws.p);
      x.key_n = (uint32_t)n;
      x.key_base = (uint32_t)b0;
      x.key_build = k == 0 && !cs;
      x.key_ready = c.keys;
      x.key_after = blob && !cs ? c.join[2] : nullptr;
      if (cr) {
        x.rdec = static_cast<const uint4*>(c.rdec.p);
        x.r_ready = c.rready;
      }
    }
    x.wide_min = (uint32_t)g_tune_wide_min.load();
    if (fault_now() || stl::launch_verify(sig + 64 * b0, msg + 32 * b0, pk + 32 * b0, cnt, words + b0 / 64, mode,
                                          false, x) != hipSuccess)
      return fail(STL_EHIP);
  }
  if (S > 1) {
    if (hipEventRecord(c.join[1], ks[1]) != hipSuccess || hipStreamWaitEvent(s, c.join[1], 0) != hipSuccess)
      return fail(STL_EHIP);
  }
  if (flag_dev && !ahead) STL_TRY(stl::launch_key_sample(pk, (uint32_t)n, flag_dev, s));
  return STL_OK;
}
}

int stl_tx_verify_batch_device(const uint8_t* d_preimages, const uint64_t* d_offset, const uint32_t* d_len,
                               const uint8_t* d_sig, const uint8_t* d_pk, size_t n, uint64_t* d_bitmap_words,
                               uint32_t flags, void* stream) {
  if (n == 0) return STL_OK;
  if (!d_preimages || !d_offset || !d_len || !d_sig || !d_pk || !d_bitmap_words) return STL_EINVAL;
  STL_RC(check_flags(flags));
  if (n > 0xffffffc0ull) return STL_EINVAL;
  Device* d = nullptr;
  STL_RC(device_for_call(&d));
  return checksign_device(*d, static_cast<hipStream_t>(stream), false, 0u, d_preimages, d_offset, d_len, d_sig, d_pk,
                          n, d_bitmap_words, nullptr, nullptr, flags);
}

int stl_signed_blob_verify_batch_device(uint32_t kind, const uint8_t* d_blobs, const uint64_t* d_offset,
                                        const uint32_t* d_len, size_t n, uint64_t* d_bitmap_words, uint8_t* d_status,
                                        uint8_t* d_id, uint32_t flags, void* stream) {
  if (kind != STL_BLOB_TRANSACTION && kind != STL_BLOB_VALIDATION) return STL_EINVAL;
  if (n == 0) return STL_OK;
  if (!d_blobs || !d_offset || !d_len || !d_bitmap_words || !d_status) return STL_EINVAL;
  STL_RC(check_flags(flags));
  if (n > 0xffffffc0ull) return STL_EINVAL;
  Device* d = nullptr;
  STL_RC(device_for_call(&d));
  return checksign_device(*d, static_cast<hipStream_t>(stream), true, kind, d_blobs, d_offset, d_len, nullptr,
                          nullptr, n, d_bitmap_words, d_status, d_id, flags);
}

int stl_ed25519_verify_batch_device(const uint8_t* d_sig, const uint8_t* d_msg, const uint8_t* d_pk, size_t n,
                                    uint64_t* d_bitmap_words, uint32_t flags, void* stream) {
  if (n == 0) return STL_OK;
  if (!d_sig || !d_msg || !d_pk || !d_bitmap_words) return STL_EINVAL;
  STL_RC(check_flags(flags));
  if (n > 0xffffffc0ull) return STL_EINVAL;
  Device* d = nullptr;
  STL_RC(device_for_call(&d));
  hipStream_t s = static_cast<hipStream_t>(stream);
  const std::shared_ptr<StreamCtx> c = stream_ctx(*d, s);
  uint32_t mode = stl::kernel_mode(flags);
  uint32_t* flag_dev = nullptr;
  STL_RC(auto_dedup_device(*c, flags, &mode, &flag_dev));
  STL_RC(run_verify(*d, s, d_sig, d_msg, d_pk, n, d_bitmap_words, mode, false, g_tune_streams.load()));
  if (flag_dev) STL_TRY(stl::launch_key_sample(d_pk, (uint32_t)n, flag_dev, s));
  return STL_OK;
}

int stl_debug_clock_stamp(uint64_t* d_out, uint32_t nwg, void* stream) {
  if (!d_out || nwg > 65536) return STL_EINVAL;
  Device* d = nullptr;
  STL_RC(device_for_call(&d));
  STL_TRY(stl::launch_clock_stamp(reinterpret_cast<unsigned long long*>(d_out), nwg,
                                  static_cast<hipStream_t>(stream)));
  return STL_OK;
}

int stl_debug_verify_k_device(const uint8_t* d_sig, const uint8_t* d_k, const uint8_t* d_pk, size_t n,
                              uint64_t* d_bitmap_words, uint32_t flags, void* stream) {
  if (n == 0) return STL_OK;
  if (!d_sig || !d_k || !d_pk || !d_bitmap_words) return STL_EINVAL;
  STL_RC(check_flags(flags));
  if (n > 0xffffffc0ull) return STL_EINVAL;
  Device* d = nullptr;
  STL_RC(device_for_call(&d));
  hipStream_t s = static_cast<hipStream_t>(stream);
  return run_verify(*d, s, d_sig, d_k, d_pk, n, d_bitmap_words, stl::kernel_mode(flags), true,
                    g_tune_streams.load());
}

int stl_tx_hash_batch_device(const uint8_t* d_preimages, const uint64_t* d_offset, const uint32_t* d_len, size_t n,
                             uint8_t* d_msg, void* stream) {
  if (n == 0) return STL_OK;
  if (!d_preimages || !d_offset || !d_len || !d_msg || n > 0xffffffc0ull) return STL_EINVAL;
  Device* d = nullptr;
  STL_RC(device_for_call(&d));
  hipStream_t s = static_cast<hipStream_t>(stream);
  const std::shared_ptr<StreamCtx> c = stream_ctx(*d, s);
  std::lock_guard<std::mutex> lk(c->mu);
  uint32_t* ctr = nullptr;
  STL_RC(ctx_queue(*c, n, &ctr));
  STL_TRY(stl::launch_tx_hash(d_preimages, d_offset, d_len, (uint32_t)n, d_msg, ctr, hash_grid(*d), s,
                              hash_long_min(*d, n)));
  return STL_OK;
}

int stl_signed_blob_prepare_device(uint32_t kind, const uint8_t* d_blobs, const uint64_t* d_offset,
                                   const uint32_t* d_len, size_t n, uint8_t* d_msg, uint8_t* d_sig, uint8_t* d_pk,
                                   uint8_t* d_id, uint8_t* d_status, void* stream) {
  if (kind != STL_BLOB_TRANSACTION && kind != STL_BLOB_VALIDATION) return STL_EINVAL;
  if (n == 0) return STL_OK;
  if (!d_blobs || !d_offset || !d_len || !d_msg || !d_sig || !d_pk || !d_status || n > 0xffffffc0ull)
    return STL_EINVAL;
  Device* d = nullptr;
  STL_RC(device_for_call(&d));
  hipStream_t s = static_cast<hipStream_t>(stream);
  const std::shared_ptr<StreamCtx> c = stream_ctx(*d, s);
  std::lock_guard<std::mutex> lk(c->mu);
  uint32_t* ctr = nullptr;
  STL_RC(ctx_queue(*c, n, &ctr, true));
  STL_TRY(stl::launch_tx_blob(d_blobs, d_offset, d_len, (uint32_t)n, d_msg, d_sig, d_pk, d_id, d_status, ctr,
                              hash_grid(*d), s, kind));
  return STL_OK;
}

int stl_tx_blob_prepare_device(const uint8_t* d_blobs, const uint64_t* d_offset, const uint32_t* d_len, size_t n,
                               uint8_t* d_msg, uint8_t* d_sig, uint8_t* d_pk, uint8_t* d_tx_id, uint8_t* d_status,
                               void* stream) {
  return stl_signed_blob_prepare_device(STL_BLOB_TRANSACTION, d_blobs, d_offset, d_len, n, d_msg, d_sig, d_pk,
                                        d_tx_id, d_status, stream);
}

int stl_ed25519_sign_batch_device(const uint8_t* d_seed, const uint8_t* d_msg, size_t n, uint8_t* d_pk,
                                  uint8_t* d_sig, void* stream) {
  if (n == 0) return STL_OK;
  if (!d_seed || !d_msg || !d_pk || !d_sig || n > 0xffffffc0ull) return STL_EINVAL;
  Device* d = nullptr;
  STL_RC(device_for_call(&d));
  hipStream_t s = static_cast<hipStream_t>(stream);
  const std::shared_ptr<StreamCtx> c = stream_ctx(*d, s);
  std::lock_guard<std::mutex> lk(c->mu);
  STL_RC(c->ws.ensure(stl::verify_ws_bytes(d->grid)));
  STL_TRY(stl::launch_sign(d_seed, d_msg, (uint32_t)n, d_pk, d_sig, static_cast<uint4*>(c->ws.p), grid_for(*d, n), s));
  return STL_OK;
}

int stl_debug_sign_adversarial_device(const uint8_t* d_seed, const uint8_t* d_msg, const uint8_t* d_cls,
                                      const uint32_t* d_param, size_t n, uint8_t* d_pk, uint8_t* d_sig,
                                      uint8_t* d_msg_out, void* stream) {
  if (n == 0) return STL_OK;
  if (!d_seed || !d_msg || !d_cls || !d_param || !d_pk || !d_sig || !d_msg_out || n > 0xffffffc0ull)
    return STL_EINVAL;
  Device* d = nullptr;
  STL_RC(device_for_call(&d));
  hipStream_t s = static_cast<hipStream_t>(stream);
  const std::shared_ptr<StreamCtx> c = stream_ctx(*d, s);
  std::lock_guard<std::mutex> lk(c->mu);
  STL_RC(c->ws.ensure(stl::verify_ws_bytes(d->grid)));
  STL_TRY(stl::launch_sign(d_seed, d_msg, (uint32_t)n, d_pk, d_sig, static_cast<uint4*>(c->ws.p), grid_for(*d, n), s,
                           d_cls, d_param, d_msg_out));
  return STL_OK;
}


int stl_comm_unique_id(uint8_t id[128]) {
  if (!id) return STL_EINVAL;
  static_assert(sizeof(ncclUniqueId) == 128, "ncclUniqueId is 128 bytes");
  if (!g_rccl.load()) return STL_ERCCL;
  ncclUniqueId u;
  STL_RCCL_TRY(g_rccl.GetUniqueId(&u));
  std::memcpy(id, &u, sizeof u);
  return STL_OK;
}

int stl_comm_init_rank(int nranks, int rank, const uint8_t id[128]) {
  if (!id || nranks < 1 || rank < 0 || rank >= nranks) return STL_EINVAL;
  Device* d = nullptr;
  STL_RC(device_for_call(&d));
  if (!g_rccl.load()) return STL_ERCCL;
  std::lock_guard<std::mutex> lk(g_pcomm_mu);
  if (g_pcomm) return STL_EINVAL;
  ncclUniqueId u;
  std::memcpy(&u, id, sizeof u);
  ncclComm_t c = nullptr;
  if (g_rccl.nonblocking()) {
    ncclConfig_t cfg = NCCL_CONFIG_INITIALIZER;
    cfg.blocking = 0;
    if (fault_now()) return STL_ERCCL;
    const ncclResult_t r = g_rccl.CommInitRankConfig(&c, nranks, u, rank, &cfg);
    const int rc = c ? rccl_settle(c, r) : STL_ERCCL;
    if (rc) {
      if (c) (void)g_rccl.CommAbort(c);
      return rc;
    }
  } else {
    STL_RCCL_TRY(g_rccl.CommInitRank(&c, nranks, u, rank));
  }
  g_pcomm = c;
  g_pcomm_ranks = nranks;
  return STL_OK;
}

void stl_comm_destroy(void) {
  std::lock_guard<std::mutex> lk(g_pcomm_mu);
  if (g_pcomm && g_rccl.ok) (void)g_rccl.CommDestroy(g_pcomm);
  g_pcomm = nullptr;
  g_pcomm_ranks = 0;
}

void stl_comm_abort(void) {
  std::lock_guard<std::mutex> lk(g_pcomm_mu);
  pcomm_abort_locked();
}

int stl_comm_sync(void* stream, int timeout_ms) {
  const hipStream_t s = static_cast<hipStream_t>(stream);
  const int ms = timeout_ms > 0 ? timeout_ms : g_rccl_timeout_ms.load();
  if (fault_now()) {
    std::lock_guard<std::mutex> lk(g_pcomm_mu);
    pcomm_abort_locked();
    return STL_ERCCL;
  }
  hipEvent_t start = nullptr;
  {
    std::lock_guard<std::mutex> lk(g_pcomm_mu);
    if (g_gather_stream == s) start = g_gather_start;
  }
  if (start) {
    const long long cap_ms = std::max<long long>(10ll * ms, g_rccl_timeout_ms.load());
    const auto cap = std::chrono::steady_clock::now() + std::chrono::milliseconds(cap_ms);
    hipError_t q;
    while ((q = hipEventQuery(start)) == hipErrorNotReady) {
      if (std::chrono::steady_clock::now() > cap) return STL_EHIP;
      std::this_thread::sleep_for(std::chrono::microseconds(50));
    }
    if (q != hipSuccess) return STL_EHIP;
  }
  const auto end = std::chrono::steady_clock::now() + std::chrono::milliseconds(ms);
  for (;;) {
    const hipError_t q = hipStreamQuery(s);
    if (q == hipSuccess) return STL_OK;
    if (q != hipErrorNotReady) return STL_EHIP;
    {
      std::lock_guard<std::mutex> lk(g_pcomm_mu);
      ncclResult_t st = ncclSuccess;
      const bool failed = g_pcomm && g_rccl.CommGetAsyncError &&
                          (g_rccl.CommGetAsyncError(g_pcomm, &st) != ncclSuccess ||
                           (st != ncclSuccess && st != ncclInProgress));
      if (failed || std::chrono::steady_clock::now() > end) {
        pcomm_abort_locked();
        return STL_ERCCL;
      }
    }
    std::this_thread::sleep_for(std::chrono::microseconds(50));
  }
}

int stl_comm_info(int* nranks, int* rank) {
  if (!nranks || !rank) return STL_EINVAL;
  {
    std::lock_guard<std::mutex> lk(g_pcomm_mu);
    if (g_pcomm) {
      STL_RCCL_TRY(g_rccl.CommCount(g_pcomm, nranks));
      STL_RCCL_TRY(g_rccl.CommUserRank(g_pcomm, rank));
      return STL_OK;
    }
  }
  std::lock_guard<std::mutex> lk(g_mu);
  if (!g_comm_gather || g_devs.empty()) return STL_ERCCL;
  int di = current_device_index();
  if (di < 0) di = 0;
  STL_RCCL_TRY(g_rccl.CommCount(g_devs[di]->comm, nranks));
  STL_RCCL_TRY(g_rccl.CommUserRank(g_devs[di]->comm, rank));
  return STL_OK;
}

int stl_bitmap_gather_device(const uint64_t* d_words, size_t words_per_rank, uint64_t* d_all_words, int root,
                             void* stream) {
  std::lock_guard<std::mutex> lk(g_pcomm_mu);
  if (!g_pcomm) return STL_ERCCL;
  if (!d_words || words_per_rank == 0 || root >= g_pcomm_ranks) return STL_EINVAL;
  hipStream_t s = static_cast<hipStream_t>(stream);
  if (root < 0 && !d_all_words) return STL_EINVAL;
  if (fault_now()) return STL_ERCCL;
  mark_gather_start(s);
  ncclResult_t r;
  if (root < 0)
    r = g_rccl.AllGather(d_words, d_all_words, words_per_rank, ncclUint64, g_pcomm, s);
  else
    r = g_rccl.Gather(d_words, d_all_words, words_per_rank, ncclUint64, root, g_pcomm, s);
  const int rc = rccl_settle(g_pcomm, r);
  if (rc) pcomm_abort_locked();
  return rc;
}

int stl_bitmap_gatherv_device(const uint64_t* d_words, size_t nwords, uint64_t* d_all_words,
                              const uint64_t* word_offsets, int root, void* stream) {
  std::lock_guard<std::mutex> lk(g_pcomm_mu);
  if (!g_pcomm) return STL_ERCCL;
  if (!word_offsets || root < 0 || root >= g_pcomm_ranks) return STL_EINVAL;
  int me = 0;
  STL_RCCL_TRY(g_rccl.CommUserRank(g_pcomm, &me));
  const int g = g_pcomm_ranks;
  for (int r = 0; r < g; ++r)
    if (word_offsets[r + 1] < word_offsets[r]) return STL_EINVAL;
  if (word_offsets[me + 1] - word_offsets[me] != nwords || (nwords && !d_words)) return STL_EINVAL;
  if (me == root && !d_all_words) return STL_EINVAL;
  hipStream_t s = static_cast<hipStream_t>(stream);
  if (me == root && nwords)
    STL_TRY(hipMemcpyAsync(d_all_words + word_offsets[me], d_words, nwords * 8, hipMemcpyDeviceToDevice, s));
  mark_gather_start(s);
  STL_RCCL_TRY(g_rccl.GroupStart());
  int rc = STL_OK;
  if (me != root) {
    if (nwords && g_rccl.Send(d_words, nwords, ncclUint64, root, g_pcomm, s) != ncclSuccess) rc = STL_ERCCL;
  } else {
    for (int r = 0; r < g; ++r) {
      const size_t w = word_offsets[r + 1] - word_offsets[r];
      if (r == root || w == 0) continue;
      if (g_rccl.Recv(d_all_words + word_offsets[r], w, ncclUint64, r, g_pcomm, s) != ncclSuccess) rc = STL_ERCCL;
    }
  }
  const int erc = rccl_settle(g_pcomm, g_rccl.GroupEnd());
  if (erc) pcomm_abort_locked();
  return rc ? rc : erc;
}

namespace {
void base_point_bytes(uint8_t out[32]) {
  std::memset(out, 0x66, 32);
  out[0] = 0x58;
}

int keyset_build(Device& d, stl_keyset& ks, std::vector<uint8_t>& all, DevBuf& dpk, DevBuf& scratch) {
  const uint32_t nk = ks.nkeys;
  STL_TRY(hipSetDevice(d.ordinal));
  STL_RC(ks.rec.ensure(((size_t)nk + 1) * stl::keyset_rec_words() * 4));
  STL_RC(ks.tables.ensure(ks.table_bytes()));
  STL_RC(dpk.ensure(((size_t)nk + 1) * 32));
  const uint32_t step = std::min<uint32_t>(nk + 1, 512);
  STL_RC(scratch.ensure((size_t)step * stl::keyset_scratch_words_per_key() * 4));
  all = ks.pk;
  all.resize(((size_t)nk + 1) * 32);
  base_point_bytes(&all[(size_t)nk * 32]);
  STL_TRY(hipMemcpyAsync(dpk.p, all.data(), all.size(), hipMemcpyHostToDevice, d.stream));
  STL_TRY(hipMemsetAsync(ks.tables.p, 0, ks.table_bytes(), d.stream));
  STL_TRY(stl::launch_keyset_decode(static_cast<const uint8_t*>(dpk.p), nk, static_cast<uint32_t*>(ks.rec.p), d.stream));
  for (uint32_t first = 0; first <= nk; first += step)
    STL_TRY(stl::launch_keyset_build(ks.d_rec(), first, std::min<uint32_t>(step, nk + 1 - first),
                                     static_cast<uint32_t*>(ks.tables.p), static_cast<uint32_t*>(scratch.p),
                                     d.stream));
// ... 181 lines not shown
```

### stellard_amd/csrc/stl_kernels.h

```cpp
#pragma once
#include <hip/hip_runtime.h>
#include <stdint.h>

namespace stl {

constexpr uint32_t kBlock = 256;
constexpr uint32_t kHeadQuads = 2 * 8 * 8;
constexpr uint32_t kSlotQuads = kHeadQuads + 2 * 9;
constexpr size_t kWsBytesPerBlock = (size_t)kBlock * kSlotQuads * 16;
constexpr uint32_t kPreChunk = 1u << 20;
constexpr uint32_t kMainQueueWords = 1u << 16;
constexpr size_t kPreBytes = (size_t)kPreChunk * 224 + (size_t)kPreChunk / 8 + (size_t)kMainQueueWords * 4;
constexpr size_t kDedupSlots = 2 * (size_t)kPreChunk;
constexpr uint32_t kKeyTables = 1u << 16;
constexpr uint32_t kWideKeys = 4096;
constexpr uint32_t kWideKeyRepeat = 32;
constexpr size_t kDedupBytes = kDedupSlots * 4 + 3 * (size_t)kPreChunk * 4 + 256 + (size_t)kPreChunk * 80 +
                               (size_t)kKeyTables * 81 * 16 + (size_t)kWideKeys * 137 * 9 * 16;
inline size_t verify_ws_bytes(uint32_t grid, bool dedup = false) {
  return kWsBytesPerBlock * grid + kPreBytes + (dedup ? kDedupBytes : 0);
}

constexpr uint32_t kModeFullLength = 0x100u;
constexpr uint32_t kModeDedupKeys = 0x200u;
constexpr uint32_t kModeOneLane = 0x400u;
constexpr uint32_t kModeRaw = 0x800u;
inline uint32_t kernel_mode(uint32_t flags) {
  return (flags & 0x1u) | ((flags & 0x4u) ? kModeFullLength : 0u) | ((flags & 0x8u) ? kModeDedupKeys : 0u) |
         ((flags & 0x10u) ? kModeOneLane : 0u) | ((flags & 0x80000000u) ? kModeRaw : 0u);
}
__host__ __device__ inline uint32_t core_policy(uint32_t mode) { return (mode & 1u) | ((mode & kModeRaw) ? 2u : 0u); }

const void* kernel_verify_msg32();
struct PhaseClock {
  void (*mark)(void* ctx, hipStream_t stream, int i);
  void* ctx;
};
constexpr uint32_t kMaxVerifyStreams = 4;
struct VerifyExec {
  uint32_t grid = 1;
  uint32_t ws_grid = 0;
  uint32_t pair_max = 0;
  const uint4* wide = nullptr;
  unsigned long long* counters = nullptr;
  const PhaseClock* clock = nullptr;
  int fused_prep = 1;
  bool main_queue = true;
  bool concurrent = false;
  uint32_t nstreams = 1;
  uint32_t sub = kPreChunk;
  uint32_t first = 0;
  hipStream_t streams[kMaxVerifyStreams] = {};
  uint4* ws[kMaxVerifyStreams] = {};
  hipEvent_t fork = nullptr;
  hipEvent_t join[kMaxVerifyStreams] = {};
  uint32_t quad_max = 0;
  uint32_t duo_max = 0;
  bool points_done = false;
  hipEvent_t key_ready = nullptr;
  hipEvent_t key_after = nullptr;
  uint4* key_ws = nullptr;
  uint32_t key_base = 0, key_n = 0;
  bool key_build = false;
  hipStream_t key_stream = nullptr;
  uint32_t wide_min = 0;
  const uint4* rdec = nullptr;
  hipEvent_t r_ready = nullptr;
};
hipError_t launch_point_r(const uint8_t* sig, const uint8_t* pk, uint32_t n, uint32_t policy, uint4* rdec,
                          hipStream_t stream);
hipError_t launch_key_domain_ws(const uint8_t* pk, uint32_t n, uint4* ws, uint32_t grid, uint32_t wide_min,
                                hipStream_t stream);
bool verify_pair_points(uint32_t n, uint32_t policy, const VerifyExec& x);
hipError_t launch_verify_points(const uint8_t* sig, const uint8_t* pk, uint32_t n, uint32_t policy,
                                const VerifyExec& x, hipStream_t stream);
hipError_t launch_verify(const uint8_t* sig, const uint8_t* msg_or_k, const uint8_t* pk, uint32_t n,
                         uint64_t* bitmap, uint32_t policy, bool pre_k, const VerifyExec& x);
hipError_t launch_hram_var(const uint8_t* sig, const uint8_t* pk, const uint8_t* m, const uint64_t* moff,
                           const uint64_t* mlen, uint32_t n, uint8_t* k_out, hipStream_t stream);
constexpr size_t kQueueHeaderBytes = 1024;
inline size_t hash_queue_bytes(size_t n) { return kQueueHeaderBytes + 4 * n; }
inline size_t blob_layout_offset(size_t n) { return (hash_queue_bytes(n) + 15) / 16 * 16; }
inline size_t blob_side_offset(size_t n) { return blob_layout_offset(n) + 32 * n; }
inline size_t blob_queue_bytes(size_t n) { return blob_side_offset(n) + 128 * n; }
hipError_t launch_tx_hash(const uint8_t* pre, const uint64_t* off, const uint32_t* len, uint32_t n, uint8_t* msg,
                          uint32_t* qws, uint32_t grid, hipStream_t stream, uint32_t long_min = 0);
hipError_t launch_tx_blob(const uint8_t* blobs, const uint64_t* off, const uint32_t* len, uint32_t n, uint8_t* msg,
                          uint8_t* sig, uint8_t* pk, uint8_t* txid, uint8_t* status, uint32_t* qws, uint32_t grid,
                          hipStream_t stream, uint32_t kind = 0u , hipEvent_t parsed = nullptr);
hipError_t launch_tx_blob_parse(const uint8_t* blobs, const uint64_t* off, const uint32_t* len, uint32_t n,
                                uint8_t* msg, uint8_t* sig, uint8_t* pk, uint8_t* txid, uint8_t* status,
                                uint32_t* qws, uint32_t grid, hipStream_t stream, uint32_t kind, hipEvent_t parsed);
hipError_t launch_tx_blob_hash(const uint8_t* blobs, const uint64_t* off, const uint32_t* len, uint32_t n,
                               uint8_t* msg, uint8_t* sig, uint8_t* pk, uint8_t* txid, uint8_t* status,
                               uint32_t* qws, uint32_t grid, hipStream_t stream, uint32_t kind);
constexpr size_t kWideTableBytes = 2ull * 32769 * 28 * 4;
hipError_t launch_key_sample(const uint8_t* pk, uint32_t n, uint32_t* flag, hipStream_t stream);
hipError_t launch_wide_table(uint4* out, hipStream_t stream);
hipError_t launch_clock_stamp(unsigned long long* out, uint32_t nwg, hipStream_t stream);
hipError_t launch_sign(const uint8_t* seed, const uint8_t* msg, uint32_t n, uint8_t* pk, uint8_t* sig, uint4* ws,
                       uint32_t grid, hipStream_t stream, const uint8_t* cls = nullptr,
                       const uint32_t* param = nullptr, uint8_t* msg_out = nullptr);

}
```

### stellard_amd/csrc/stl_kernels.hip

```cpp
#include "stl_base_table.h"
#include "stl_kernels.h"
#include "stl_sign.h"
#include "stl_txblob.h"
#include "stl_verify_core.h"

#ifndef STL_VERIFY_WAVES_PER_SIMD
#define STL_VERIFY_WAVES_PER_SIMD 2
#endif
#ifndef STL_PRE_WAVES_PER_SIMD
#define STL_PRE_WAVES_PER_SIMD 4
#endif
#ifndef STL_SCALAR_WAVES_PER_SIMD
#define STL_SCALAR_WAVES_PER_SIMD 4
#endif
#ifndef STL_HASH_WAVES_PER_SIMD
#define STL_HASH_WAVES_PER_SIMD 4
#endif

namespace stl {

__device__ __forceinline__ void ld8(uint32_t w[8], const uint8_t* p) {
  const uint4* q = reinterpret_cast<const uint4*>(p);
  const uint4 a = q[0], b = q[1];
  w[0] = a.x; w[1] = a.y; w[2] = a.z; w[3] = a.w;
// ... 1543 lines not shown
#pragma unroll
        for (int j = 0; j < 4; ++j) {
          h[2 * j] = bswap32((uint32_t)(st[j] >> 32));
          h[2 * j + 1] = bswap32((uint32_t)st[j]);
        }
        if (phase == 0) {
          st8(msg + 32 * (size_t)mi, h);
          if (txid != nullptr) {
            bs.init(b - pfx_bytes, len[mi] + pfx_bytes);
            nb = bs.blocks();
            blk = 0;
            sha512_init(st);
            phase = 1;
          } else {
            active = false;
          }
        } else {
          st8(txid + 32 * (size_t)mi, h);
          active = false;
        }
      }
    }
  }
}

template <bool ADV>
__global__ __launch_bounds__(kBlock, 2) void sign_kernel(const uint8_t* __restrict__ seed,
                                                      const uint8_t* __restrict__ msg, uint32_t n,
                                                      uint8_t* __restrict__ pk_out, uint8_t* __restrict__ sig_out,
                                                      uint4* __restrict__ ws, const uint8_t* __restrict__ cls,
                                                      const uint32_t* __restrict__ param,
                                                      uint8_t* __restrict__ msg_out) {
  __shared__ uint32_t sB[kBaseTableWords];
  stage_base_table(sB, 1);
  TableView tv, unused;
  lane_tables(ws, tv, unused);
  for (uint32_t base = blockIdx.x * kBlock; base < n; base += gridDim.x * kBlock) {
    const uint32_t i = base + threadIdx.x;
    const bool live = i < n;
    const size_t j = live ? i : (n - 1);
    uint32_t sd[8], M[8], A[8], R[8], S[8], a[8], r[8];
    ld8(sd, seed + 32 * j);
    ld8(M, msg + 32 * j);
    sign_row(A, R, S, a, r, sd, M, tv, sB);
    if (ADV) {
      const uint32_t c = cls[j];
      if (c != 0) adversarial_row(c, param[j], A, R, S, M, a, r, tv, sB);
    }
    if (live) {
      st8(pk_out + 32 * j, A);
      st8(sig_out + 64 * j, R);
      st8(sig_out + 64 * j + 32, S);
      if (ADV) st8(msg_out + 32 * j, M);
    }
  }
}

const void* kernel_verify_msg32() { return reinterpret_cast<const void*>(&verify_main_kernel<false>); }

__global__ __launch_bounds__(kBlock) void wide_table_kernel(uint32_t* __restrict__ out) {
  const uint32_t r = blockIdx.x * kBlock + threadIdx.x;
  if (r >= 2 * kWideEntries) return;
  const int which = r >= kWideEntries ? 1 : 0;
  uint32_t row[28];
  wide_entry(row, which, r - (uint32_t)which * kWideEntries, &kBaseNiels[0][0][0]);
  const uint32_t* src = row;
  uint4* q = reinterpret_cast<uint4*>(out) + (size_t)r * kWideQuads;
#pragma unroll
  for (int c = 0; c < kWideQuads; ++c) q[c] = make_uint4(src[4 * c], src[4 * c + 1], src[4 * c + 2], src[4 * c + 3]);
}

hipError_t launch_wide_table(uint4* out, hipStream_t stream) {
  hipLaunchKernelGGL(wide_table_kernel, dim3((2 * kWideEntries + kBlock - 1) / kBlock), dim3(kBlock), 0, stream,
                     reinterpret_cast<uint32_t*>(out));
  return hipGetLastError();
}

static bool pair_chunk(uint32_t cnt, uint32_t policy, const VerifyExec& x) {
  return (policy & kModeOneLane) == 0 && cnt <= x.pair_max && 2ull * cnt <= (uint64_t)x.grid * kBlock;
}

static bool pair_point_chunk(uint32_t cnt, uint32_t policy, const VerifyExec& x) {
  const bool dedup = (policy & kModeDedupKeys) != 0;
  return pair_chunk(cnt, policy, x) ||
         (!x.concurrent && (policy & kModeOneLane) == 0 && !dedup && cnt <= 2ull * x.pair_max);
}

bool verify_pair_points(uint32_t n, uint32_t policy, const VerifyExec& x) {
  return n > 0 && n <= kPreChunk && pair_point_chunk(n, policy, x);
}

hipError_t launch_verify_points(const uint8_t* sig, const uint8_t* pk, uint32_t n, uint32_t policy,
                                const VerifyExec& x, hipStream_t stream) {
  if (!verify_pair_points(n, policy, x)) return hipErrorInvalidValue;
  uint4* pre = x.ws[0] + (size_t)x.grid * (kWsBytesPerBlock / 16);
  const dim3 gp((2 * n + kBlock - 1) / kBlock);
  hipLaunchKernelGGL(verify_prep_pair_kernel<false>, gp, dim3(kBlock), 0, stream, sig, nullptr, pk, 0u, n, policy,
                     pre, 0u);
  return hipGetLastError();
}

struct KeyDomain {
  uint32_t *kslots, *rep, *uid_of, *owners, *counter;
  uint4 *keytab, *keytabs, *widetabs;
};
static KeyDomain key_domain(uint4* ws, uint32_t grid) {
  KeyDomain k;
  uint32_t* dd = reinterpret_cast<uint32_t*>(reinterpret_cast<uint8_t*>(ws) + verify_ws_bytes(grid));
  k.kslots = dd;
  k.rep = k.kslots + kDedupSlots;
  k.uid_of = k.rep + kPreChunk;
  k.owners = k.uid_of + kPreChunk;
  k.counter = k.owners + kPreChunk;
  k.keytab = reinterpret_cast<uint4*>(k.counter + 64);
  k.keytabs = k.keytab + (size_t)kPreChunk * 5;
  k.widetabs = k.keytabs + (size_t)kKeyTables * kTableQuadsPerKey;
  return k;
}

static hipError_t launch_key_domain(const uint8_t* pk, uint32_t base, uint32_t cnt, uint32_t wcnt,
                                    const KeyDomain& kd, hipStream_t stream) {
  const dim3 g1((cnt + kBlock - 1) / kBlock);
  uint32_t nslots = 64;
  while (nslots < 2 * cnt) nslots <<= 1;
  hipError_t e = hipMemsetAsync(kd.kslots, 0xff, (size_t)nslots * 4, stream);
  if (e != hipSuccess) return e;
  e = hipMemsetAsync(kd.counter, 0, 4, stream);
  if (e != hipSuccess) return e;
  hipLaunchKernelGGL(key_insert_kernel, g1, dim3(kBlock), 0, stream, pk, base, cnt, kd.kslots, nslots - 1, kd.rep,
                     kd.uid_of, kd.counter, kd.owners);
  hipLaunchKernelGGL(key_decode_kernel, g1, dim3(kBlock), 0, stream, pk, base, kd.counter, kd.owners, kd.keytab,
                     kd.keytabs, wcnt);
  const uint32_t wmax = wcnt / kWideKeyRepeat < kWideKeys ? wcnt / kWideKeyRepeat : kWideKeys;
  if (wmax > 0) {
    hipLaunchKernelGGL(key_table_wide_base_kernel, dim3((wmax * (uint32_t)kWideBaseEntries + kBlock - 1) / kBlock),
                       dim3(kBlock), 0, stream, kd.counter, wcnt, kd.keytab, kd.widetabs);
    hipLaunchKernelGGL(key_table_wide_pair_kernel, dim3((wmax * (uint32_t)kWideKeyEntries + kBlock - 1) / kBlock),
                       dim3(kBlock), 0, stream, kd.counter, wcnt, kd.widetabs);
  }
  return hipGetLastError();
}

static uint32_t wide_count(uint32_t cnt, uint32_t wide_min) { return cnt >= wide_min ? cnt : 0u; }

hipError_t launch_key_domain_ws(const uint8_t* pk, uint32_t n, uint4* ws, uint32_t grid, uint32_t wide_min,
                                hipStream_t stream) {
  if (n == 0 || n > kPreChunk) return hipErrorInvalidValue;
  return launch_key_domain(pk, 0, n, wide_count(n, wide_min), key_domain(ws, grid), stream);
}

static hipError_t verify_chunk(const uint8_t* sig, const uint8_t* msg_or_k, const uint8_t* pk, uint32_t base,
                               uint32_t cnt, uint64_t* bitmap, uint32_t policy, bool pre_k, const VerifyExec& x,
                               hipStream_t stream, uint4* ws, uint32_t* qctr, const PhaseClock* clock) {
  const uint32_t grid = x.grid, pair_max = x.pair_max;
  const uint4* wide = x.wide;
  unsigned long long* counters = x.counters;
  auto mark = [&](int i) {
    if (clock) clock->mark(clock->ctx, stream, i);
  };
  uint4* slots = ws;
  uint4* pre = ws + (size_t)grid * (kWsBytesPerBlock / 16);
  uint64_t* fb = reinterpret_cast<uint64_t*>(pre + (size_t)kPreChunk * 14);
  const bool dedup = (policy & kModeDedupKeys) != 0;
  const KeyDomain kd = key_domain(x.key_ws ? x.key_ws : ws, x.ws_grid ? x.ws_grid : grid);
  uint32_t* kslots = kd.kslots;
  uint32_t* rep = x.key_ws ? kd.rep + x.key_base + base : kd.rep;
  uint32_t* uid_of = kd.uid_of;
  uint32_t* owners = kd.owners;
  uint32_t* counter = kd.counter;
  uint4* keytab = kd.keytab;
  uint4* keytabs = kd.keytabs;
  uint4* widetabs = kd.widetabs;
  const uint32_t kcnt = wide_count(x.key_ws ? x.key_n : cnt, x.wide_min);
  {
    const dim3 g1((cnt + kBlock - 1) / kBlock);
    const uint32_t units = (cnt + 63) / 64;
    const uint32_t wgs = (units + kBlock / 64 - 1) / (kBlock / 64);
    const dim3 g2(wgs < grid ? wgs : grid);
    const bool pair = pair_chunk(cnt, policy, x);
    const bool pair_point = pair_point_chunk(cnt, policy, x);
    const dim3 gp((2 * cnt + kBlock - 1) / kBlock);
    const bool fused = x.fused_prep != 0 && !pair_point && !dedup;
    mark(0);
    if (pair_point) {
      const uint32_t nbs = (cnt + kBlock - 1) / kBlock;
      const uint32_t nblk = nbs + (x.points_done ? 0u : gp.x);
      if (pre_k)
        hipLaunchKernelGGL(verify_prep_pair_kernel<true>, dim3(nblk), dim3(kBlock), 0, stream, sig, msg_or_k, pk,
                           base, cnt, policy, pre, nbs);
      else
        hipLaunchKernelGGL(verify_prep_pair_kernel<false>, dim3(nblk), dim3(kBlock), 0, stream, sig, msg_or_k,
                           pk, base, cnt, policy, pre, nbs);
    } else if (fused && pre_k)
      hipLaunchKernelGGL(verify_prep_kernel<true>, g1, dim3(kBlock), 0, stream, sig, msg_or_k, pk, base, cnt, policy,
                         pre, fb);
    else if (fused)
      hipLaunchKernelGGL(verify_prep_kernel<false>, g1, dim3(kBlock), 0, stream, sig, msg_or_k, pk, base, cnt, policy,
                         pre, fb);
    else if (pre_k)
      hipLaunchKernelGGL(verify_scalar_kernel<true>, g1, dim3(kBlock), 0, stream, sig, msg_or_k, pk, base, cnt, pre);
    else
      hipLaunchKernelGGL(verify_scalar_kernel<false>, g1, dim3(kBlock), 0, stream, sig, msg_or_k, pk, base, cnt, pre);
    mark(1);
    if (pair_point) {
      if (!pair)
        hipLaunchKernelGGL(verify_finish_pair_kernel, g1, dim3(kBlock), 0, stream, cnt, policy, pre, fb);
    } else if (fused) {
    } else if (dedup) {
      if (!x.key_ws) {
        hipError_t e = launch_key_domain(pk, base, cnt, kcnt, kd, stream);
        if (e != hipSuccess) return e;
      } else if (x.key_build) {
        hipError_t e = x.key_after ? hipStreamWaitEvent(stream, x.key_after, 0) : hipSuccess;
        if (e == hipSuccess) e = launch_key_domain(pk, 0, x.key_n, kcnt, kd, stream);
        if (e == hipSuccess) e = hipEventRecord(x.key_ready, stream);
        if (e != hipSuccess) return e;
      } else {
        hipError_t e = hipStreamWaitEvent(stream, x.key_ready, 0);
        if (e != hipSuccess) return e;
      }
      if (x.key_ws && x.rdec) {
        hipError_t e = hipStreamWaitEvent(stream, x.r_ready, 0);
        if (e != hipSuccess) return e;
        hipLaunchKernelGGL(verify_finish_keyed_kernel, g1, dim3(kBlock), 0, stream, cnt, policy, pre, fb, rep, uid_of,
                           keytab, counter, kcnt, x.rdec + (size_t)(x.key_base + base) * 5);
      } else {
        hipLaunchKernelGGL(verify_point_kernel_keyed, g1, dim3(kBlock), 0, stream, sig, pk, base, cnt, policy, pre,
                           fb, rep, uid_of, keytab, counter, kcnt);
      }
    } else {
      hipLaunchKernelGGL(verify_point_kernel, g1, dim3(kBlock), 0, stream, sig, pk, base, cnt, policy, pre, fb);
    }
    mark(2);
    const uint32_t words = (cnt + 63) / 64;
    const bool fits = pair && words <= 2 * grid;
    if (fits && cnt <= x.quad_max)
      hipLaunchKernelGGL(verify_main_group_kernel<4>, dim3(2 * words), dim3(kBlock), 0, stream, pre, base, cnt, policy,
                         bitmap, fb, slots, wide, counters);
    else if (fits && cnt <= x.duo_max)
      hipLaunchKernelGGL(verify_main_group_kernel<2>, dim3(words), dim3(kBlock), 0, stream, pre, base, cnt, policy,
                         bitmap, fb, slots, wide, counters);
    else if (pair)
      hipLaunchKernelGGL(verify_main_pair_kernel, gp, dim3(kBlock), 0, stream, pre, base, cnt, policy, bitmap, fb,
                         slots, wide, counters);
    else if (!dedup)
      hipLaunchKernelGGL(verify_main_kernel<true>, g2, dim3(kBlock), 0, stream, pre, base, cnt, bitmap, slots, wide,
                         counters, nullptr, nullptr, qctr);
    else
      hipLaunchKernelGGL(verify_main_kernel<false>, g2, dim3(kBlock), 0, stream, pre, base, cnt, bitmap, slots, wide,
                         counters, dedup ? keytabs : nullptr, dedup ? widetabs : nullptr, qctr);
    mark(3);
    if (pre_k)
      hipLaunchKernelGGL(verify_fallback_kernel<true>, g2, dim3(kBlock), 0, stream, sig, msg_or_k, pk, base, cnt,
                         policy, fb, bitmap, slots, counters);
    else
      hipLaunchKernelGGL(verify_fallback_kernel<false>, g2, dim3(kBlock), 0, stream, sig, msg_or_k, pk, base, cnt,
                         policy, fb, bitmap, slots, counters);
    mark(4);
  }
  return hipGetLastError();
}

static uint32_t* queue_counters(uint4* ws, uint32_t grid) {
  uint4* pre = ws + (size_t)grid * (kWsBytesPerBlock / 16);
  return reinterpret_cast<uint32_t*>(reinterpret_cast<uint64_t*>(pre + (size_t)kPreChunk * 14) + kPreChunk / 64);
}

hipError_t launch_verify(const uint8_t* sig, const uint8_t* msg_or_k, const uint8_t* pk, uint32_t n,
                         uint64_t* bitmap, uint32_t policy, bool pre_k, const VerifyExec& x) {
  if (n == 0) return hipSuccess;
  uint32_t S = x.nstreams < kMaxVerifyStreams ? x.nstreams : kMaxVerifyStreams;
  const uint32_t sub = x.sub;
  if (S > 1 && (x.clock != nullptr || sub > kPreChunk || (sub & 63u) != 0 || n <= sub ||
                ((uint64_t)n + sub - 1) / sub > (uint64_t)kMainQueueWords))
    S = 1;
  const uint32_t csize = S > 1 ? sub : kPreChunk;
  const uint32_t first = S > 1 && x.first && (x.first & 63u) == 0 && x.first < csize && x.first < n ? x.first : 0u;
  const uint64_t nchunks = first ? 1 + ((uint64_t)(n - first) + csize - 1) / csize : ((uint64_t)n + csize - 1) / csize;
  if (S > (uint32_t)nchunks) S = (uint32_t)nchunks;
  if (x.points_done && (nchunks != 1 || !verify_pair_points(n, policy, x))) return hipErrorInvalidValue;
  hipError_t e;
  if (S > 1) {
    if ((e = hipEventRecord(x.fork, x.streams[0])) != hipSuccess) return e;
    for (uint32_t j = 1; j < S; ++j)
      if ((e = hipStreamWaitEvent(x.streams[j], x.fork, 0)) != hipSuccess) return e;
  }
  if (x.main_queue && !(nchunks == 1 && pair_chunk(n, policy, x))) {
    for (uint32_t j = 0; j < S; ++j) {
      const uint64_t cj = (nchunks - j + S - 1) / S;
      e = hipMemsetAsync(queue_counters(x.ws[j], x.grid), 0, cj * 4, x.streams[j]);
      if (e != hipSuccess) return e;
    }
  }
  VerifyExec xk = x;
  const bool shared_keys = (policy & kModeDedupKeys) && nchunks > 1 && n <= kPreChunk && x.key_ready &&
                           !x.key_ws && csize > x.pair_max &&
                           (first == 0 || first > x.pair_max);
  if (shared_keys) {
    xk.key_ws = x.ws[0];
    xk.key_base = 0;
    xk.key_n = n;
    if (x.key_stream) {
      e = S > 1 ? hipStreamWaitEvent(x.key_stream, x.fork, 0) : hipSuccess;
      if (e == hipSuccess)
        e = launch_key_domain(pk, 0, n, wide_count(n, x.wide_min),
                              key_domain(x.ws[0], x.ws_grid ? x.ws_grid : x.grid), x.key_stream);
      if (e == hipSuccess) e = hipEventRecord(x.key_ready, x.key_stream);
      if (e != hipSuccess) return e;
    }
  }
  for (uint64_t c = 0; c < nchunks; ++c) {
    const uint32_t j = (uint32_t)(c % S);
    const uint32_t base = first ? (c == 0 ? 0u : (uint32_t)(first + (c - 1) * csize)) : (uint32_t)(c * csize);
    const uint32_t cap = first && c == 0 ? first : csize;
    const uint32_t cnt = n - base < cap ? n - base : cap;
    uint32_t* q = x.main_queue ? queue_counters(x.ws[j], x.grid) + c / S : nullptr;
    if (shared_keys) xk.key_build = c == 0 && !x.key_stream;
    e = verify_chunk(sig, msg_or_k, pk, base, cnt, bitmap, policy, pre_k, xk, x.streams[j], x.ws[j], q,
                     S > 1 ? nullptr : x.clock);
    if (e != hipSuccess) return e;
  }
  if (S > 1) {
    for (uint32_t j = 1; j < S; ++j) {
      if ((e = hipEventRecord(x.join[j], x.streams[j])) != hipSuccess) return e;
      if ((e = hipStreamWaitEvent(x.streams[0], x.join[j], 0)) != hipSuccess) return e;
    }
  }
  return hipGetLastError();
}

hipError_t launch_hram_var(const uint8_t* sig, const uint8_t* pk, const uint8_t* m, const uint64_t* moff,
                           const uint64_t* mlen, uint32_t n, uint8_t* k_out, hipStream_t stream) {
  if (n == 0) return hipSuccess;
  hipLaunchKernelGGL(hram_var_kernel, dim3((n + 63) / 64), dim3(64), 0, stream, sig, pk, m, moff, mlen, n, k_out);
  return hipGetLastError();
}

static hipError_t launch_order(const uint32_t* len, uint32_t n, uint32_t extra, uint32_t* qws, hipStream_t stream,
                               uint32_t long_min = 0) {
  hipError_t e = hipMemsetAsync(qws, 0, kQueueHeaderBytes, stream);
  if (e != hipSuccess) return e;
  uint32_t* hist = qws + 64;
  uint32_t* cursor = qws + 128;
  uint32_t* order = qws + kQueueHeaderBytes / 4;
  const uint32_t tiles = (n + kBlock - 1) / kBlock;
  const uint32_t grid = tiles < 1024u ? tiles : 1024u;
  hipLaunchKernelGGL(order_count_kernel, dim3(grid), dim3(kBlock), 0, stream, len, n, extra, hist);
  hipLaunchKernelGGL(order_scan_kernel, dim3(1), dim3(64), 0, stream, hist, cursor, qws, long_min);
  hipLaunchKernelGGL(order_scatter_kernel, dim3(grid), dim3(kBlock), 0, stream, len, n, extra, cursor, order);
  return hipGetLastError();
}

hipError_t launch_tx_hash(const uint8_t* pre, const uint64_t* off, const uint32_t* len, uint32_t n, uint8_t* msg,
                          uint32_t* qws, uint32_t grid, hipStream_t stream, uint32_t long_min) {
  if (n == 0) return hipSuccess;
  hipError_t e = launch_order(len, n, 0u, qws, stream, long_min);
  if (e != hipSuccess) return e;
  uint32_t blocks = (n + kBlock - 1) / kBlock;
  if (blocks > grid) blocks = grid;
  if (long_min) blocks += kLongMaxRows / (kBlock / 64u);
  hipLaunchKernelGGL(tx_hash_kernel, dim3(blocks), dim3(kBlock), 0, stream, pre, off, len, n, msg, qws,
                     qws + kQueueHeaderBytes / 4);
  return hipGetLastError();
}

hipError_t launch_tx_blob_parse(const uint8_t* blobs, const uint64_t* off, const uint32_t* len, uint32_t n,
                                uint8_t* msg, uint8_t* sig, uint8_t* pk, uint8_t* txid, uint8_t* status,
                                uint32_t* qws, uint32_t grid, hipStream_t stream, uint32_t kind_id,
                                hipEvent_t parsed) {
  if (n == 0) return hipSuccess;
  const BlobKind kind = kind_id == 1u ? blob_kind_validation() : blob_kind_tx();
  uint4* layout = reinterpret_cast<uint4*>(reinterpret_cast<uint8_t*>(qws) + blob_layout_offset(n));
  uint4* side = reinterpret_cast<uint4*>(reinterpret_cast<uint8_t*>(qws) + blob_side_offset(n));
  const uint32_t blocks = (n + kBlock - 1) / kBlock;
  const uint32_t pgrid = 2u * grid;
  hipLaunchKernelGGL(tx_blob_parse_kernel, dim3(blocks < pgrid ? blocks : pgrid), dim3(kBlock), 0, stream, blobs, off,
                     len, n, msg, sig, pk, txid, status, layout, side, kind);
  hipError_t e = hipGetLastError();
  if (e == hipSuccess && parsed) e = hipEventRecord(parsed, stream);
  return e;
}

hipError_t launch_tx_blob_hash(const uint8_t* blobs, const uint64_t* off, const uint32_t* len, uint32_t n,
                               uint8_t* msg, uint8_t* sig, uint8_t* pk, uint8_t* txid, uint8_t* status,
                               uint32_t* qws, uint32_t grid, hipStream_t stream, uint32_t kind_id) {
  if (n == 0) return hipSuccess;
  const BlobKind kind = kind_id == 1u ? blob_kind_validation() : blob_kind_tx();
  uint4* layout = reinterpret_cast<uint4*>(reinterpret_cast<uint8_t*>(qws) + blob_layout_offset(n));
  uint4* side = reinterpret_cast<uint4*>(reinterpret_cast<uint8_t*>(qws) + blob_side_offset(n));
  const uint32_t blocks = (n + kBlock - 1) / kBlock;
  hipError_t e = launch_order(len, n, kind.id_prefixed ? 4u : 0u, qws, stream);
  if (e != hipSuccess) return e;
  hipLaunchKernelGGL(tx_blob_kernel, dim3(blocks < grid ? blocks : grid), dim3(kBlock), 0, stream, blobs, off, len,
                     n, msg, sig, pk, txid, status, qws, qws + kQueueHeaderBytes / 4, layout, side, kind);
  return hipGetLastError();
}

hipError_t launch_tx_blob(const uint8_t* blobs, const uint64_t* off, const uint32_t* len, uint32_t n, uint8_t* msg,
                          uint8_t* sig, uint8_t* pk, uint8_t* txid, uint8_t* status, uint32_t* qws, uint32_t grid,
                          hipStream_t stream, uint32_t kind_id, hipEvent_t parsed) {
  hipError_t e = launch_tx_blob_parse(blobs, off, len, n, msg, sig, pk, txid, status, qws, grid, stream, kind_id,
                                      parsed);
  if (e != hipSuccess) return e;
  return launch_tx_blob_hash(blobs, off, len, n, msg, sig, pk, txid, status, qws, grid, stream, kind_id);
}

hipError_t launch_sign(const uint8_t* seed, const uint8_t* msg, uint32_t n, uint8_t* pk, uint8_t* sig, uint4* ws,
                       uint32_t grid, hipStream_t stream, const uint8_t* cls, const uint32_t* param,
                       uint8_t* msg_out) {
  if (n == 0) return hipSuccess;
  if (cls)
    hipLaunchKernelGGL(sign_kernel<true>, dim3(grid), dim3(kBlock), 0, stream, seed, msg, n, pk, sig, ws, cls, param,
                       msg_out);
  else
    hipLaunchKernelGGL(sign_kernel<false>, dim3(grid), dim3(kBlock), 0, stream, seed, msg, n, pk, sig, ws, nullptr,
                       nullptr, nullptr);
  return hipGetLastError();
}

}
```

Before: 126.8 million.

## Plan host-to-device uploads per chunk and gate verify launches on upload events

After: 126.6 million. About the same (-0.1%).

```diff
diff --git a/stellard_amd/build.py b/stellard_amd/build.py
--- a/stellard_amd/build.py
+++ b/stellard_amd/build.py
@@ -11,7 +11,7 @@
 PRODUCT_SRCS = ["stl_kernels.hip", "stl_keyset.hip", "stl_api.cpp", "stl_batcher.cpp"]
 PRODUCT_DEPS = PRODUCT_SRCS + ["stl_kernels.h", "stl_verify_core.h", "stl_fe25519.h", "stl_ge25519.h",
                                "stl_sc25519.h", "stl_sha512.h", "stl_base_table.h", "stl_lattice.h", "stl_txblob.h", "stl_sign.h",
-                               "stl_comb.h", "stl_keyset.h",
+                               "stl_comb.h", "stl_keyset.h", "stl_upload_plan.h",
                                os.path.join("..", "..", "include", "stl.h")]
 
 
@@ -36,7 +36,7 @@
     subprocess.run(cmd, cwd=cwd, check=True)
 
 
-HOST_DEPS = ["stl_kernels.h", "stl_keyset.h", os.path.join("..", "..", "include", "stl.h")]
+HOST_DEPS = ["stl_kernels.h", "stl_keyset.h", "stl_upload_plan.h", os.path.join("..", "..", "include", "stl.h")]
 OBJ_DIR = os.path.join(ROOT, "build", "obj")
 
 
diff --git a/stellard_amd/csrc/stl_api.cpp b/stellard_amd/csrc/stl_api.cpp
--- a/stellard_amd/csrc/stl_api.cpp
+++ b/stellard_amd/csrc/stl_api.cpp
@@ -20,6 +20,7 @@
 #include "../../include/stl.h"
 #include "stl_kernels.h"
 #include "stl_keyset.h"
+#include "stl_upload_plan.h"
 
 namespace {
 
@@ -238,6 +239,10 @@
 std::atomic<int> g_tune_wide_min{0};
 std::atomic<int> g_tune_r_ahead{1};
 std::atomic<int> g_tune_first_chunk{0};
+std::atomic<int> g_feed_chunk_log2{16};
+std::atomic<int> g_feed_first{0};
+std::atomic<int> g_feed_piece_log2{26};
+std::atomic<int> g_feed_key_stream{1};
 
 std::atomic<uint64_t> g_shard_quantum{65536};
 
@@ -380,6 +385,7 @@
   std::mutex ws_mu;
   void* stage = nullptr;
   size_t stage_cap = 0;
+  std::vector<hipEvent_t> feed_ev;
   PhaseTimer timer;
   stl::PhaseClock clock{phase_mark, &timer};
 };
@@ -511,6 +517,8 @@
   if (d.stage) (void)hipHostFree(d.stage);
   d.stage = nullptr;
   d.stage_cap = 0;
+  for (hipEvent_t e : d.feed_ev) (void)hipEventDestroy(e);
+  d.feed_ev.clear();
   d.timer.release();
   for (hipStream_t s : {d.stream, d.stream2, s3, d.copy})
     if (s) (void)hipStreamDestroy(s);
@@ -620,8 +628,93 @@
   return nullptr;
 }
 
+int pool_stream3(Device& d, hipStream_t* out) {
+  if (!d.stream3.load()) {
+    std::lock_guard<std::mutex> lk(d.ws_mu);
+    if (!d.stream3.load()) {
+      hipStream_t s3 = nullptr;
+      STL_TRY(hipStreamCreateWithFlags(&s3, hipStreamNonBlocking));
+      d.stream3.store(s3);
+    }
+  }
+  *out = d.stream3.load();
+  return STL_OK;
+}
+
+struct Feed {
+  Device* d = nullptr;
+  const uint8_t* src[stl::kUploadBufs] = {};
+  uint8_t* dst[stl::kUploadBufs] = {};
+  const uint64_t* roff = nullptr;
+  const uint32_t* len = nullptr;
+  stl::UploadShape shape;
+  stl::UploadPlan plan;
+  size_t issued = 0;
+  struct Mark {
+    int32_t piece;
+    hipEvent_t ev;
+  };
+  std::vector<Mark> marks;
+  size_t ev_used = 0;
+  std::pair<hipStream_t, int32_t> waits[stl::kMaxVerifyStreams + 1] = {};
+  size_t nwaits = 0;
+  stl::RowsFeed hook{&Feed::ready, this};
+  Feed() = default;
+  Feed(const Feed&) = delete;
+  Feed& operator=(const Feed&) = delete;
+
+  int begin() {
+    shape.piece_bytes = shape.first_piece_bytes = (uint64_t)1 << g_feed_piece_log2.load();
+    return stl::plan_upload(shape, roff, len, &plan) == stl::kPlanOk ? STL_OK : STL_EINVAL;
+  }
+  int need(uint32_t kind, uint64_t row0, uint64_t rows, hipStream_t consumer) {
+    int32_t last = (int32_t)plan.pieces.size() - 1;
+    for (const stl::UploadStage& st : plan.stages)
+      if (st.kind == kind && st.row0 == row0 && st.rows == rows) {
+        last = st.last;
+        break;
+      }
+    if (last < 0) return STL_OK;
+    for (; issued <= (size_t)last; ++issued) {
+      const stl::UploadPiece& p = plan.pieces[issued];
+      STL_TRY(hipMemcpyAsync(dst[p.buf] + p.at, src[p.buf] + p.at, p.bytes, hipMemcpyHostToDevice, d->copy));
+    }
+    if (consumer == d->copy) return STL_OK;
+    for (size_t i = 0; i < nwaits; ++i)
+      if (waits[i].first == consumer && waits[i].second >= last) return STL_OK;
+    hipEvent_t ev = nullptr;
+    int32_t upto = 0;
+    for (const Mark& m : marks)
+      if (!ev && m.piece >= last) {
+        ev = m.ev;
+        upto = m.piece;
+      }
+    if (!ev) {
+      if (ev_used == d->feed_ev.size()) {
+        hipEvent_t e = nullptr;
+        STL_TRY(hipEventCreateWithFlags(&e, hipEventDisableTiming));
+        d->feed_ev.push_back(e);
+      }
+      ev = d->feed_ev[ev_used++];
+      STL_TRY(hipEventRecord(ev, d->copy));
+      upto = (int32_t)issued - 1;
+      marks.push_back(Mark{upto, ev});
+    }
+    STL_TRY(hipStreamWaitEvent(consumer, ev, 0));
+    size_t w = 0;
+    while (w < nwaits && waits[w].first != consumer) ++w;
+    if (w == nwaits && nwaits < sizeof waits / sizeof waits[0]) ++nwaits;
+    if (w < nwaits) waits[w] = {consumer, upto};
+    return STL_OK;
+  }
+  static hipError_t ready(void* ctx, uint32_t what, uint32_t row0, uint32_t rows, hipStream_t stream) {
+    return static_cast<Feed*>(ctx)->need(what, row0, rows, stream) == STL_OK ? hipSuccess : hipErrorUnknown;
+  }
+  bool complete() const { return issued == plan.pieces.size(); }
+};
+
 int run_verify(Device& d, hipStream_t s, const uint8_t* sig, const uint8_t* msg_or_k, const uint8_t* pk, size_t n,
-               uint64_t* words, uint32_t mode, bool pre_k, int streams, bool concurrent = false) {
+               uint64_t* words, uint32_t mode, bool pre_k, int streams, bool concurrent = false, Feed* up = nullptr) {
   const bool dedup = (mode & stl::kModeDedupKeys) != 0;
   stl::VerifyExec x;
   x.grid = verify_grid_for(d, n);
@@ -637,19 +730,24 @@
   x.concurrent = concurrent;
   x.sub = chunk_for(d.grid, n);
   x.first = (uint32_t)g_tune_first_chunk.load();
+  if (up) {
+    const int cl = g_feed_chunk_log2.load();
+    if (cl && !g_tune_sub_log2.load() && n > ((size_t)1 << cl)) {
+      x.sub = 1u << cl;
+      x.concurrent = true;
+    }
+    const uint32_t ff = (uint32_t)g_feed_first.load();
+    if (ff && !x.first && x.sub >= 2 * ff) x.first = ff;
+  }
   uint32_t S = (uint32_t)std::max(1, std::min<int>(streams, (int)stl::kMaxVerifyStreams));
   if (x.clock || n <= x.sub || x.sub <= x.pair_max) S = 1;
   S = (uint32_t)std::min<size_t>(S, (n + x.sub - 1) / x.sub);
   hipStream_t pool[stl::kMaxVerifyStreams] = {s};
   uint32_t np = 1;
   if (S > 1) {
-    if (S > 3 && !d.stream3.load()) {
-      std::lock_guard<std::mutex> lk(d.ws_mu);
-      if (!d.stream3.load()) {
-        hipStream_t s3 = nullptr;
-        STL_TRY(hipStreamCreateWithFlags(&s3, hipStreamNonBlocking));
-        d.stream3.store(s3);
-      }
+    if (S > 3) {
+      hipStream_t s3 = nullptr;
+      STL_RC(pool_stream3(d, &s3));
     }
     for (hipStream_t p : {d.stream2, d.stream, d.stream3.load()})
       if (np < S && p && p != s) pool[np++] = p;
@@ -684,6 +782,22 @@
     if (!c.keys) STL_TRY(hipEventCreateWithFlags(&c.keys, hipEventDisableTiming));
     x.key_ready = c.keys;
     x.key_stream = key_stream_for(d, pool, S);
+  }
+  if (up) {
+    stl::UploadShape& sh = up->shape;
+    sh.sub = S > 1 ? x.sub : stl::kPreChunk;
+    sh.first = S > 1 && x.first && (x.first & 63u) == 0 && x.first < sh.sub && x.first < n ? x.first : 0;
+    const uint64_t nchunks = stl::upload_chunks(sh);
+    sh.keys_stage = dedup && nchunks > 1 && n <= stl::kPreChunk && x.key_ready && sh.sub > x.pair_max &&
+                    (sh.first == 0 || sh.first > x.pair_max);
+    sh.key_domain = dedup;
+    sh.key_off = stl::verify_ws_bytes(x.ws_grid);
+    sh.key_bytes = stl::kDedupBytes;
+    sh.key_max_rows = stl::kPreChunk;
+    sh.ws_cap = ctx[0]->ws.cap;
+    for (uint32_t j = 1; j < S; ++j) sh.ws_cap = std::min<uint64_t>(sh.ws_cap, ctx[j]->ws.cap);
+    STL_RC(up->begin());
+    x.feed = &up->hook;
   }
   if (fault_now() || stl::launch_verify(sig, msg_or_k, pk, (uint32_t)n, words, mode, pre_k, x) != hipSuccess) {
     for (uint32_t j = 1; j < S; ++j) (void)hipStreamSynchronize(pool[j]);
@@ -749,11 +863,6 @@
   }
 }
 
-#ifndef STL_PIPE_CHUNK_LOG2
-#define STL_PIPE_CHUNK_LOG2 16
-#endif
-constexpr size_t kPipeChunk = (size_t)1 << STL_PIPE_CHUNK_LOG2;
-
 enum class Mode { kSig, kPre, kBlob };
 
 struct Batch {
@@ -799,53 +908,49 @@
 
 uint32_t chunk_policy(const Batch& b, size_t lo, size_t hi) {
   if (!b.auto_dedup || !keys_repeat(b, lo, hi)) return b.policy;
-  g_st_auto_dedup++;
+  g_st_auto_dedup += (hi - lo + 65535) / 65536;
   return b.policy | stl::kModeDedupKeys;
 }
 
 struct Shard {
   Device* d = nullptr;
   size_t lo = 0, hi = 0;
-  std::vector<uint64_t> roff, row_end;
-  std::vector<hipEvent_t> ev;
+  std::vector<uint64_t> roff;
+  size_t st_words = 0, st_status = 0, st_id = 0;
   int rc = STL_OK;
-  ~Shard() {
-    for (hipEvent_t e : ev) (void)hipEventDestroy(e);
-  }
-  int join(hipStream_t from, hipStream_t to) {
-    hipEvent_t e;
-    STL_TRY(hipEventCreateWithFlags(&e, hipEventDisableTiming));
-    ev.push_back(e);
-    STL_TRY(hipEventRecord(e, from));
-    STL_TRY(hipStreamWaitEvent(to, e, 0));
-    return STL_OK;
-  }
 };
 
-void rebase(const uint64_t* off, const uint32_t* len, size_t lo, size_t hi, std::vector<uint64_t>& roff,
-            std::vector<uint64_t>& row_end, uint64_t* base_out, uint64_t* bytes_out) {
-  const size_t n = hi - lo;
-  uint64_t base = off[lo], end = 0;
-  for (size_t i = lo; i < hi; ++i) base = std::min(base, off[i]);
-  roff.resize(n);
-  row_end.resize(n);
-  for (size_t i = 0; i < n; ++i) {
-    roff[i] = off[lo + i] - base;
-    row_end[i] = roff[i] + len[lo + i];
-    end = std::max(end, row_end[i]);
-  }
+int span(const uint64_t* off, const uint32_t* len, size_t lo, size_t hi, uint64_t* base_out, uint64_t* bytes_out) {
+  uint64_t base = UINT64_MAX, end = 0, over = 0;
+  for (size_t i = lo; i < hi; ++i) {
+    const uint64_t e = off[i] + len[i];
+    over |= e < off[i];
+    base = std::min(base, off[i]);
+    end = std::max(end, e);
+  }
+  if (over) return STL_EINVAL;
   *base_out = base;
-  *bytes_out = end;
-}
-
-int copy_rows(Shard& s, uint8_t* dst, const uint8_t* src, size_t c0, size_t c1, uint64_t* watermark) {
-  uint64_t need = *watermark;
-  for (size_t i = c0; i < c1; ++i) need = std::max(need, s.row_end[i]);
-  if (need > *watermark)
-    STL_TRY(hipMemcpyAsync(dst + *watermark, src + *watermark, need - *watermark, hipMemcpyHostToDevice, s.d->copy));
-  *watermark = need;
-  return STL_OK;
-}
+  *bytes_out = end - base;
+  return STL_OK;
+}
+
+int stage_ensure(Device& d, size_t bytes) {
+  if (d.stage_cap >= bytes) return STL_OK;
+  if (d.stage) (void)hipHostFree(d.stage);
+  d.stage = nullptr;
+  d.stage_cap = 0;
+  const size_t cap = std::max<size_t>(bytes, 4096 * 128 + 4096 / 8);
+  if (fault_now() || hipHostMalloc(&d.stage, cap, hipHostMallocDefault) != hipSuccess) {
+    d.stage = nullptr;
+    return STL_ENOMEM;
+  }
+  d.stage_cap = cap;
+  return STL_OK;
+}
+
+int checksign_device(Device& d, hipStream_t s, bool blob, uint32_t kind, const uint8_t* bytes, const uint64_t* off,
+                     const uint32_t* len, const uint8_t* sig_in, const uint8_t* pk_in, size_t n, uint64_t* words,
+                     uint8_t* status, uint8_t* id, uint32_t flags, Feed* up, uint32_t up_mode);
 
 int enqueue_shard(const Batch& b, Shard& s, size_t words_alloc) {
   Device& d = *s.d;
@@ -853,76 +958,113 @@
   STL_TRY(hipSetDevice(d.ordinal));
   STL_RC(d.bitmap.ensure(std::max<size_t>(words_alloc, 1) * 8));
   if (n == 0) return STL_OK;
-  STL_RC(d.sig.ensure(n * 64));
-  STL_RC(d.msg.ensure(n * 32));
-  STL_RC(d.pk.ensure(n * 32));
-  uint64_t base = 0, bytes = 0, mark = 0;
+  const bool blob = b.mode == Mode::kBlob;
+  if (!blob) {
+    STL_RC(d.sig.ensure(n * 64));
+    STL_RC(d.pk.ensure(n * 32));
+  }
+  if (b.mode == Mode::kSig) STL_RC(d.msg.ensure(n * 32));
+  uint64_t base = 0;
+  const uint64_t* roff = nullptr;
+  if (b.mode != Mode::kSig) {
+    uint64_t bytes = 0;
+    STL_RC(span(b.off, b.len, lo, s.hi, &base, &bytes));
+    if (base == 0) {
+      roff = b.off + lo;
+    } else {
+      s.roff.resize(n);
+      for (size_t i = 0; i < n; ++i) s.roff[i] = b.off[lo + i] - base;
+      roff = s.roff.data();
+    }
+    STL_RC(d.pre.ensure(bytes + 16));
+    STL_RC(d.off.ensure(n * 8));
+    STL_RC(d.len.ensure(n * 4));
+    if (blob) {
+      STL_RC(d.status.ensure(n));
+      if (b.txid) STL_RC(d.txid.ensure(n * 32));
+    }
+  }
+  const size_t wbytes = (n + 63) / 64 * 8;
+  s.st_words = 0;
+  s.st_status = wbytes;
+  s.st_id = (wbytes + n + 63) / 64 * 64;
+  STL_RC(stage_ensure(d, s.st_id + (blob && b.txid ? n * 32 : 0)));
   uint8_t* dsig = static_cast<uint8_t*>(d.sig.p);
   uint8_t* dmsg = static_cast<uint8_t*>(d.msg.p);
   uint8_t* dpk = static_cast<uint8_t*>(d.pk.p);
-  uint8_t* dpre = nullptr;
-  uint64_t* doff = nullptr;
-  uint32_t* dlen = nullptr;
-  if (b.mode != Mode::kSig) {
-    rebase(b.off, b.len, lo, s.hi, s.roff, s.row_end, &base, &bytes);
-    STL_RC(d.pre.ensure(bytes + 16));
-    STL_RC(d.off.ensure(n * 8));
-    STL_RC(d.len.ensure(n * 4));
-    const size_t qn = std::min(n, kPipeChunk);
-    const size_t qbytes = b.mode == Mode::kBlob ? stl::blob_queue_bytes(qn) : stl::hash_queue_bytes(qn);
-    STL_RC(d.ctr.ensure(qbytes));
-    if (b.mode == Mode::kBlob) {
-      STL_RC(d.status.ensure(n));
-      if (b.txid) STL_RC(d.txid.ensure(n * 32));
-    }
-    dpre = static_cast<uint8_t*>(d.pre.p);
-    doff = static_cast<uint64_t*>(d.off.p);
-    dlen = static_cast<uint32_t*>(d.len.p);
-    STL_TRY(hipMemcpyAsync(doff, s.roff.data(), n * 8, hipMemcpyHostToDevice, d.copy));
-    STL_TRY(hipMemcpyAsync(dlen, b.len + lo, n * 4, hipMemcpyHostToDevice, d.copy));
-  }
-  uint8_t* dtxid = (b.mode == Mode::kBlob && b.txid) ? static_cast<uint8_t*>(d.txid.p) : nullptr;
-  uint8_t* dstatus = b.mode == Mode::kBlob ? static_cast<uint8_t*>(d.status.p) : nullptr;
-  const bool two = g_tune_streams.load() > 1 && n > kPipeChunk && !phase_clock(d);
-  if (b.auto_dedup && n > kPipeChunk / 2)
-    for (hipStream_t ks : {d.stream, d.stream2}) {
-      const std::shared_ptr<StreamCtx> c = stream_ctx(d, ks);
-      std::lock_guard<std::mutex> lk(c->mu);
-      STL_RC(c->ws.ensure(stl::verify_ws_bytes(d.grid, true)));
-    }
-  if (two && b.mode != Mode::kSig) {
-    const size_t qn = std::min(n, kPipeChunk);
-    STL_RC(d.ctr2.ensure(b.mode == Mode::kBlob ? stl::blob_queue_bytes(qn) : stl::hash_queue_bytes(qn)));
-  }
-  for (size_t c0 = 0; c0 < n; c0 += kPipeChunk) {
-    const size_t c1 = std::min(n, c0 + kPipeChunk), cn = c1 - c0;
-    const bool odd = two && ((c0 / kPipeChunk) & 1);
-    hipStream_t ks = odd ? d.stream2 : d.stream;
-    uint32_t* kctr = static_cast<uint32_t*>((odd ? d.ctr2 : d.ctr).p);
-    if (b.mode != Mode::kBlob) {
-      STL_TRY(hipMemcpyAsync(dsig + 64 * c0, b.sig + 64 * (lo + c0), cn * 64, hipMemcpyHostToDevice, d.copy));
-      STL_TRY(hipMemcpyAsync(dpk + 32 * c0, b.pk + 32 * (lo + c0), cn * 32, hipMemcpyHostToDevice, d.copy));
-    }
+  uint8_t* dpre = static_cast<uint8_t*>(d.pre.p);
+  uint64_t* doff = static_cast<uint64_t*>(d.off.p);
+  uint32_t* dlen = static_cast<uint32_t*>(d.len.p);
+  uint64_t* dwords = static_cast<uint64_t*>(d.bitmap.p);
+  uint8_t* dtxid = (blob && b.txid) ? static_cast<uint8_t*>(d.txid.p) : nullptr;
+  uint8_t* dstatus = blob ? static_cast<uint8_t*>(d.status.p) : nullptr;
+  uint64_t bytes_up = 0;
+  size_t ev_used = 0;
+  if (b.mode != Mode::kSig && g_feed_key_stream.load()) {
+    hipStream_t s3 = nullptr;
+    STL_RC(pool_stream3(d, &s3));
+  }
+  for (size_t g0 = 0; g0 < n; g0 += stl::kPreChunk) {
+    const size_t gn = std::min<size_t>(n - g0, stl::kPreChunk);
+    Feed up;
+    up.d = &d;
+    up.ev_used = ev_used;
+    stl::UploadShape& sh = up.shape;
+    sh.mode = b.mode == Mode::kSig ? stl::kUploadSig : blob ? stl::kUploadBlob : stl::kUploadPre;
+    sh.n = gn;
+    auto bind = [&](uint32_t buf, const void* src, void* dst, size_t cap_bytes, size_t at) {
+      up.src[buf] = static_cast<const uint8_t*>(src) + at;
+      up.dst[buf] = static_cast<uint8_t*>(dst) + at;
+      sh.cap[buf] = cap_bytes - at;
+    };
+    if (!blob) {
+      bind(stl::kBufSig, b.sig + 64 * lo, dsig, d.sig.cap, 64 * g0);
+      bind(stl::kBufPk, b.pk + 32 * lo, dpk, d.pk.cap, 32 * g0);
+    }
+    if (b.mode == Mode::kSig) {
+      bind(stl::kBufMsg, b.msg32 + 32 * lo, dmsg, d.msg.cap, 32 * g0);
+    } else {
+      bind(stl::kBufOff, roff, doff, d.off.cap, 8 * g0);
+      bind(stl::kBufLen, b.len + lo, dlen, d.len.cap, 4 * g0);
+      bind(stl::kBufBytes, b.bytes + base, dpre, d.pre.cap, 0);
+      sh.from[stl::kBufBytes] = bytes_up;
+      up.roff = roff + g0;
+      up.len = b.len + lo + g0;
+    }
+    sh.out_cap[0] = d.bitmap.cap - g0 / 8;
+    sh.out_need[0] = (gn + 63) / 64 * 8;
+    if (blob) {
+      sh.out_cap[1] = d.status.cap - g0;
+      sh.out_need[1] = gn;
+      if (dtxid) {
+        sh.out_cap[2] = d.txid.cap - 32 * g0;
+        sh.out_need[2] = 32 * gn;
+      }
+    }
+    const uint32_t mode = chunk_policy(b, lo + g0, lo + g0 + gn);
     if (b.mode == Mode::kSig)
-      STL_TRY(hipMemcpyAsync(dmsg + 32 * c0, b.msg32 + 32 * (lo + c0), cn * 32, hipMemcpyHostToDevice, d.copy));
+      STL_RC(run_verify(d, d.stream, dsig + 64 * g0, dmsg + 32 * g0, dpk + 32 * g0, gn, dwords + g0 / 64, mode, false,
+                        g_tune_streams.load(), false, &up));
     else
-      STL_RC(copy_rows(s, dpre, b.bytes + base, c0, c1, &mark));
-    STL_RC(s.join(d.copy, ks));
-    if (b.mode == Mode::kPre)
-      STL_TRY(stl::launch_tx_hash(dpre, doff + c0, dlen + c0, (uint32_t)cn, dmsg + 32 * c0, kctr, hash_grid(d), ks,
-                                  hash_long_min(d, n)));
-    else if (b.mode == Mode::kBlob)
-      STL_TRY(stl::launch_tx_blob(dpre, doff + c0, dlen + c0, (uint32_t)cn, dmsg + 32 * c0, dsig + 64 * c0,
-                                  dpk + 32 * c0, dtxid ? dtxid + 32 * c0 : nullptr, dstatus + c0, kctr,
-                                  hash_grid(d), ks, b.kind));
-    STL_RC(run_verify(d, ks, dsig + 64 * c0, dmsg + 32 * c0, dpk + 32 * c0, cn,
-                      static_cast<uint64_t*>(d.bitmap.p) + c0 / 64, chunk_policy(b, lo + c0, lo + c1), false, 1,
-                      two));
-  }
-  if (two) STL_RC(s.join(d.stream2, d.stream));
-  if (dstatus && b.status) STL_TRY(hipMemcpyAsync(b.status + lo, dstatus, n, hipMemcpyDeviceToHost, d.stream));
-  if (dtxid) STL_TRY(hipMemcpyAsync(b.txid + 32 * lo, dtxid, n * 32, hipMemcpyDeviceToHost, d.stream));
-  return STL_OK;
+      STL_RC(checksign_device(d, d.stream, blob, b.kind, dpre, doff + g0, dlen + g0,
+                              blob ? nullptr : dsig + 64 * g0, blob ? nullptr : dpk + 32 * g0, gn, dwords + g0 / 64, blob ? dstatus + g0 : nullptr, dtxid ? dtxid + 32 * g0 : nullptr,
+                              0u, &up, mode));
+    if (!up.complete()) return STL_EHIP;
+    bytes_up = up.plan.end[stl::kBufBytes];
+    ev_used = up.ev_used;
+  }
+  uint8_t* st = static_cast<uint8_t*>(d.stage);
+  if (dstatus && b.status) STL_TRY(hipMemcpyAsync(st + s.st_status, dstatus, n, hipMemcpyDeviceToHost, d.stream));
+  if (dtxid) STL_TRY(hipMemcpyAsync(st + s.st_id, dtxid, n * 32, hipMemcpyDeviceToHost, d.stream));
+  return STL_OK;
+}
+
+void deliver(const Batch& b, const Shard& s) {
+  const size_t n = s.hi - s.lo;
+  if (n == 0 || b.mode != Mode::kBlob) return;
+  const uint8_t* st = static_cast<const uint8_t*>(s.d->stage);
+  if (b.status) std::memcpy(b.status + s.lo, st + s.st_status, n);
+  if (b.txid) std::memcpy(b.txid + 32 * s.lo, st + s.st_id, n * 32);
 }
 
 int drain(Device& d) {
@@ -935,22 +1077,22 @@
   return (a == hipSuccess && b == hipSuccess && c == hipSuccess && e == hipSuccess) ? STL_OK : STL_EHIP;
 }
 
-int finish_direct(const Batch& b, Shard& s, std::vector<uint8_t>& host_words) {
+int finish_direct(const Batch& b, Shard& s) {
   const size_t n = s.hi - s.lo;
   if (n == 0) return STL_OK;
-  host_words.resize((n + 63) / 64 * 8);
-  STL_TRY(hipMemcpyAsync(host_words.data(), s.d->bitmap.p, host_words.size(), hipMemcpyDeviceToHost, s.d->stream));
+  uint8_t* st = static_cast<uint8_t*>(s.d->stage);
+  STL_TRY(hipMemcpyAsync(st + s.st_words, s.d->bitmap.p, (n + 63) / 64 * 8, hipMemcpyDeviceToHost, s.d->stream));
   STL_TRY(hipStreamSynchronize(s.d->stream));
-  std::memcpy(b.bitmap + s.lo / 8, host_words.data(), (n + 7) / 8);
+  std::memcpy(b.bitmap + s.lo / 8, st + s.st_words, (n + 7) / 8);
+  deliver(b, s);
   return STL_OK;
 }
 
 int run_shard_direct(const Batch& b, Shard& s) {
   std::lock_guard<std::mutex> lk(s.d->mu);
   int rc = enqueue_shard(b, s, (s.hi - s.lo + 63) / 64);
-  std::vector<uint8_t> host_words;
-  if (rc == STL_OK) rc = finish_direct(b, s, host_words);
-  const int drc = drain(*s.d);
+  if (rc == STL_OK) rc = finish_direct(b, s);
+  const int drc = rc ? drain(*s.d) : STL_OK;
   return rc ? rc : drc;
 }
 
@@ -1007,17 +1149,7 @@
   std::lock_guard<std::mutex> lk(d.mu);
   STL_TRY(hipSetDevice(d.ordinal));
   const size_t bytes = n * 128, words = (n + 63) / 64;
-  if (d.stage_cap < bytes + words * 8) {
-    if (d.stage) (void)hipHostFree(d.stage);
-    d.stage = nullptr;
-    d.stage_cap = 0;
-    const size_t cap = kSmallBatch * 128 + kSmallBatch / 8;
-    if (fault_now() || hipHostMalloc(&d.stage, cap, hipHostMallocDefault) != hipSuccess) {
-      d.stage = nullptr;
-      return STL_ENOMEM;
-    }
-    d.stage_cap = cap;
-  }
+  STL_RC(stage_ensure(d, bytes + words * 8));
   STL_RC(d.sig.ensure(bytes));
   STL_RC(d.bitmap.ensure(words * 8));
   uint8_t* st = static_cast<uint8_t*>(d.stage);
@@ -1088,6 +1220,8 @@
       const int drc = drain(*d);
       rc = rc ? rc : drc;
     }
+    if (rc == STL_OK)
+      for (auto& s : sh) deliver(b, s);
     return rc;
   }
   std::vector<std::thread> th;
@@ -1158,6 +1292,12 @@
     const int ws = env_int("STL_MAX_STREAM_WORKSPACES", 0);
     if (ws >= 1 && ws <= 64) g_max_caller_streams.store(ws);
     if (c >= 15 && c <= 20) g_tune_sub_log2.store(c);
+    const int uf = env_int("STL_UPLOAD_FIRST_ROWS", -1), upl = env_int("STL_UPLOAD_PIECE_LOG2", 0);
+    const int ucl = env_int("STL_UPLOAD_CHUNK_LOG2", -1);
+    if (ucl == 0 || (ucl >= 16 && ucl <= 18)) g_feed_chunk_log2.store(ucl);
+    if (uf >= 0 && uf % 64 == 0 && uf <= (1 << 19)) g_feed_first.store(uf);
+    if (upl >= 16 && upl <= 28) g_feed_piece_log2.store(upl);
+    g_feed_key_stream.store(env_int("STL_UPLOAD_KEY_STREAM", 1) != 0);
   }
   int first = 0, want = -1, spd = 1;
   uint32_t cflags = 0;
@@ -1572,7 +1712,7 @@
 namespace {
 int checksign_device(Device& d, hipStream_t s, bool blob, uint32_t kind, const uint8_t* bytes, const uint64_t* off,
                      const uint32_t* len, const uint8_t* sig_in, const uint8_t* pk_in, size_t n, uint64_t* words,
-                     uint8_t* status, uint8_t* id, uint32_t flags) {
+                     uint8_t* status, uint8_t* id, uint32_t flags, Feed* up, uint32_t up_mode) {
   const stl::PhaseClock* clock = phase_clock(d);
   size_t sub = chunk_for(d.grid, n);
   uint32_t S = (uint32_t)std::max(1, std::min(g_tune_streams.load(), 2));
@@ -1585,9 +1725,9 @@
                                               S > 1 ? stream_ctx(d, ks[1]) : std::shared_ptr<StreamCtx>()};
   StreamCtx* kc[2] = {hold[0].get(), hold[1].get()};
   StreamCtx& c = *kc[0];
-  uint32_t mode = stl::kernel_mode(flags);
+  uint32_t mode = up ? up_mode : stl::kernel_mode(flags);
   uint32_t* flag_dev = nullptr;
-  STL_RC(auto_dedup_device(c, flags, &mode, &flag_dev));
+  if (!up) STL_RC(auto_dedup_device(c, flags, &mode, &flag_dev));
   const bool dedup = (mode & stl::kModeDedupKeys) != 0;
   auto exec_for = [&](uint32_t cnt, uint32_t j) {
     stl::VerifyExec x;
@@ -1625,16 +1765,47 @@
   for (uint32_t j = 0; j < S; ++j) STL_RC(kc[j]->ws.ensure(stl::verify_ws_bytes(d.grid, dedup)));
   const bool shared_keys = dedup && S > 1 && n <= stl::kPreChunk && sub > pair_max(d) && g_tune_shared_keys.load();
   hipStream_t cs = shared_keys ? key_stream_for(d, ks, S) : nullptr;
+  if (shared_keys && !cs && up && g_feed_key_stream.load()) cs = d.stream3.load();
   if (shared_keys && !c.keys) STL_TRY(hipEventCreateWithFlags(&c.keys, hipEventDisableTiming));
   if (cs && blob)
     for (hipEvent_t& e : c.parsed)
       if (!e) STL_TRY(hipEventCreateWithFlags(&e, hipEventDisableTiming));
   hipStream_t cr = cs && g_tune_r_ahead.load() && d.copy != cs && d.copy != ks[0] && d.copy != ks[1] ? d.copy
                                                                                                       : nullptr;
+  const size_t last_rows = n - (n - 1) / sub * sub;
+  const bool last_pairs = n > sub && !(mode & stl::kModeOneLane) && last_rows <= pair_max(d);
+  const size_t r_rows = cr ? (last_pairs ? n - last_rows : n) : 0;
   if (cr) {
     STL_RC(c.rdec.ensure(n * 80));
     if (!c.rready) STL_TRY(hipEventCreateWithFlags(&c.rready, hipEventDisableTiming));
   }
+  if (up) {
+    stl::UploadShape& sh = up->shape;
+    sh.sub = sub;
+    sh.hash_launches = S > 1 ? 2 : 1;
+    sh.keys_stage = shared_keys;
+    sh.r_rows = r_rows;
+    sh.points_ahead = ahead;
+    sh.scratch_cap = c.scratch.cap;
+    sh.scratch_row = row;
+    sh.rdec_cap = c.rdec.cap;
+    sh.key_domain = dedup;
+    sh.key_off = stl::verify_ws_bytes(d.grid);
+    sh.key_bytes = stl::kDedupBytes;
+    sh.key_max_rows = shared_keys ? stl::kPreChunk : n;
+    sh.ws_cap = kc[0]->ws.cap;
+    if (S > 1) sh.ws_cap = std::min<uint64_t>(sh.ws_cap, kc[1]->ws.cap);
+    sh.queue_cap[0] = kc[0]->queue.cap;
+    sh.queue_need[0] = blob ? stl::blob_queue_bytes(S > 1 ? sub : n) : stl::hash_queue_bytes(S > 1 ? sub : n);
+    if (S > 1) {
+      sh.queue_cap[1] = kc[1]->queue.cap;
+      sh.queue_need[1] = blob ? stl::blob_queue_bytes(n - sub) : stl::hash_queue_bytes(n - sub);
+    }
+    STL_RC(up->begin());
+  }
+  auto fed = [&](uint32_t kind, size_t row0, size_t rows, hipStream_t js) -> int {
+    return up ? up->need(kind, row0, rows, js) : STL_OK;
+  };
   if (S > 1 || ahead) {
     if (!c.fork) STL_TRY(hipEventCreateWithFlags(&c.fork, hipEventDisableTiming));
     if (!c.join[1]) STL_TRY(hipEventCreateWithFlags(&c.join[1], hipEventDisableTiming));
@@ -1649,7 +1820,8 @@
     return rc;
   };
   if (ahead) {
-    int rc = STL_OK;
+    int rc = fed(stl::kStageVerify, 0, n, ks[1]);
+    if (rc) return fail(rc);
     if (fault_now() || stl::launch_verify_points(sig, pk, (uint32_t)n, mode, exec_for((uint32_t)n, 0), ks[1]) !=
                            hipSuccess)
       rc = STL_EHIP;
@@ -1659,6 +1831,7 @@
   }
   const bool split_pass = blob && cs && S > 1;
   auto parse = [&](size_t b0, size_t cnt, hipStream_t js, uint32_t* qw) -> int {
+    STL_RC(fed(stl::kStageRows, b0, cnt, js));
     if (fault_now()) return STL_EHIP;
     const hipError_t e = stl::launch_tx_blob_parse(bytes, off + b0, len + b0, (uint32_t)cnt, msg + 32 * b0,
                                                    sig + 64 * b0, pk + 32 * b0, id ? id + 32 * b0 : nullptr, st + b0,
@@ -1667,6 +1840,7 @@
   };
   auto hash = [&](size_t b0, size_t cnt, hipStream_t js, uint32_t* qw) -> int {
     hipError_t e;
+    STL_RC(fed(stl::kStageRows, b0, cnt, js));
     if (split_pass) {
       e = stl::launch_tx_blob_hash(bytes, off + b0, len + b0, (uint32_t)cnt, msg + 32 * b0, sig + 64 * b0,
                                    pk + 32 * b0, id ? id + 32 * b0 : nullptr, st + b0, qw, hash_grid(d), js, kind);
@@ -1688,13 +1862,15 @@
       if (!rc && ahead && hipStreamWaitEvent(s, c.join[2], 0) != hipSuccess) rc = STL_EHIP;
       return rc;
     }
-    int rc = hash(0, sub, ks[0], q[0]);
+    int rc = split_pass && up ? STL_OK : hash(0, sub, ks[0], q[0]);
     if (!rc) rc = hash(sub, n - sub, ks[1], q[1]);
     if (!rc && hipEventRecord(c.join[2], ks[1]) != hipSuccess) rc = STL_EHIP;
     return rc;
   };
   if (split_pass) {
     int rc = parse(0, sub, ks[0], q[0]);
+    if (!rc && up) rc = fed(stl::kStageRows, sub, n - sub, ks[1]);
+    if (!rc && up) rc = hash(0, sub, ks[0], q[0]);
     if (!rc) rc = parse(sub, n - sub, ks[1], q[1]);
     if (rc) return fail(rc);
   } else if (int rc = hash_all()) {
@@ -1707,6 +1883,7 @@
       if (e == hipSuccess) e = hipStreamWaitEvent(cs, c.parsed[1], 0);
     } else {
       e = hipStreamWaitEvent(cs, c.fork, 0);
+      if (e == hipSuccess && fed(stl::kStageKeys, 0, n, cs)) e = hipErrorUnknown;
     }
     if (e == hipSuccess && fault_now()) e = hipErrorUnknown;
     if (e == hipSuccess)
@@ -1722,11 +1899,9 @@
       if (e == hipSuccess) e = hipStreamWaitEvent(cr, c.parsed[1], 0);
     } else {
       e = hipStreamWaitEvent(cr, c.fork, 0);
+      if (e == hipSuccess && fed(stl::kStageR, 0, r_rows, cr)) e = hipErrorUnknown;
     }
     if (e == hipSuccess && fault_now()) e = hipErrorUnknown;
-    const size_t last = n - (n - 1) / sub * sub;
-    const bool last_pairs = n > sub && !(mode & stl::kModeOneLane) && last <= pair_max(d);
-    const size_t r_rows = last_pairs ? n - last : n;
     if (e == hipSuccess)
       e = stl::launch_point_r(sig, pk, (uint32_t)r_rows, mode, static_cast<uint4*>(c.rdec.p), cr);
     if (e == hipSuccess) e = hipEventRecord(c.rready, cr);
@@ -1755,6 +1930,11 @@
       }
     }
     x.wide_min = (uint32_t)g_tune_wide_min.load();
+    if (!blob) {
+      if (x.key_build)
+        if (int rc = fed(stl::kStageKeys, 0, n, js)) return fail(rc);
+      if (int rc = fed(stl::kStageVerify, b0, cnt, js)) return fail(rc);
+    }
     if (fault_now() || stl::launch_verify(sig + 64 * b0, msg + 32 * b0, pk + 32 * b0, cnt, words + b0 / 64, mode,
                                           false, x) != hipSuccess)
       return fail(STL_EHIP);
@@ -1778,7 +1958,7 @@
   Device* d = nullptr;
   STL_RC(device_for_call(&d));
   return checksign_device(*d, static_cast<hipStream_t>(stream), false, 0u, d_preimages, d_offset, d_len, d_sig, d_pk,
-                          n, d_bitmap_words, nullptr, nullptr, flags);
+                          n, d_bitmap_words, nullptr, nullptr, flags, nullptr, 0u);
 }
 
 int stl_signed_blob_verify_batch_device(uint32_t kind, const uint8_t* d_blobs, const uint64_t* d_offset,
@@ -1792,7 +1972,7 @@
   Device* d = nullptr;
   STL_RC(device_for_call(&d));
   return checksign_device(*d, static_cast<hipStream_t>(stream), true, kind, d_blobs, d_offset, d_len, nullptr,
-                          nullptr, n, d_bitmap_words, d_status, d_id, flags);
+                          nullptr, n, d_bitmap_words, d_status, d_id, flags, nullptr, 0u);
 }
 
 int stl_ed25519_verify_batch_device(const uint8_t* d_sig, const uint8_t* d_msg, const uint8_t* d_pk, size_t n,
diff --git a/stellard_amd/csrc/stl_kernels.h b/stellard_amd/csrc/stl_kernels.h
--- a/stellard_amd/csrc/stl_kernels.h
+++ b/stellard_amd/csrc/stl_kernels.h
@@ -37,6 +37,11 @@
   void* ctx;
 };
 constexpr uint32_t kMaxVerifyStreams = 4;
+constexpr uint32_t kFeedVerify = 1, kFeedKeys = 2;
+struct RowsFeed {
+  hipError_t (*ready)(void* ctx, uint32_t what, uint32_t row0, uint32_t rows, hipStream_t stream);
+  void* ctx;
+};
 struct VerifyExec {
   uint32_t grid = 1;
   uint32_t ws_grid = 0;
@@ -66,6 +71,7 @@
   uint32_t wide_min = 0;
   const uint4* rdec = nullptr;
   hipEvent_t r_ready = nullptr;
+  const RowsFeed* feed = nullptr;
 };
 hipError_t launch_point_r(const uint8_t* sig, const uint8_t* pk, uint32_t n, uint32_t policy, uint4* rdec,
                           hipStream_t stream);
diff --git a/stellard_amd/csrc/stl_kernels.hip b/stellard_amd/csrc/stl_kernels.hip
--- a/stellard_amd/csrc/stl_kernels.hip
+++ b/stellard_amd/csrc/stl_kernels.hip
@@ -1869,6 +1869,7 @@
     xk.key_n = n;
     if (x.key_stream) {
       e = S > 1 ? hipStreamWaitEvent(x.key_stream, x.fork, 0) : hipSuccess;
+      if (e == hipSuccess && x.feed) e = x.feed->ready(x.feed->ctx, kFeedKeys, 0, n, x.key_stream);
       if (e == hipSuccess)
         e = launch_key_domain(pk, 0, n, wide_count(n, x.wide_min),
                               key_domain(x.ws[0], x.ws_grid ? x.ws_grid : x.grid), x.key_stream);
@@ -1883,6 +1884,11 @@
     const uint32_t cnt = n - base < cap ? n - base : cap;
     uint32_t* q = x.main_queue ? queue_counters(x.ws[j], x.grid) + c / S : nullptr;
     if (shared_keys) xk.key_build = c == 0 && !x.key_stream;
+    if (x.feed) {
+      e = shared_keys && xk.key_build ? x.feed->ready(x.feed->ctx, kFeedKeys, 0, n, x.streams[j]) : hipSuccess;
+      if (e == hipSuccess) e = x.feed->ready(x.feed->ctx, kFeedVerify, base, cnt, x.streams[j]);
+      if (e != hipSuccess) return e;
+    }
     e = verify_chunk(sig, msg_or_k, pk, base, cnt, bitmap, policy, pre_k, xk, x.streams[j], x.ws[j], q,
                      S > 1 ? nullptr : x.clock);
     if (e != hipSuccess) return e;
diff --git a/stellard_amd/csrc/stl_upload_plan.h b/stellard_amd/csrc/stl_upload_plan.h
--- /dev/null
+++ b/stellard_amd/csrc/stl_upload_plan.h
@@ -0,0 +1,175 @@
+#pragma once
+#include <stddef.h>
+#include <stdint.h>
+
+#include <algorithm>
+#include <initializer_list>
+#include <vector>
+
+namespace stl {
+
+enum UploadMode : uint32_t { kUploadSig = 0, kUploadPre = 1, kUploadBlob = 2 };
+enum UploadBuf : uint32_t { kBufOff = 0, kBufLen, kBufBytes, kBufSig, kBufMsg, kBufPk, kUploadBufs };
+enum UploadStageKind : uint32_t {
+  kStageRows = 0,
+  kStageVerify,
+  kStageKeys,
+  kStageR
+};
+
+struct UploadPiece {
+  uint32_t buf;
+  uint64_t at, bytes;
+};
+struct UploadStage {
+  uint32_t kind;
+  uint64_t row0, rows;
+  int32_t last;
+};
+
+struct UploadShape {
+  uint32_t mode = kUploadSig;
+  uint64_t n = 0;
+  uint64_t sub = 0;
+  uint64_t first = 0;
+  uint32_t hash_launches = 1;
+  bool keys_stage = false;
+  uint64_t r_rows = 0;
+  bool points_ahead = false;
+  uint64_t cap[kUploadBufs] = {}, from[kUploadBufs] = {};
+  uint64_t out_cap[3] = {}, out_need[3] = {};
+  uint64_t scratch_cap = 0, scratch_row = 0;
+  uint64_t rdec_cap = 0, rdec_row = 80;
+  bool key_domain = false;
+  uint64_t ws_cap = 0, key_off = 0, key_bytes = 0, key_max_rows = 0;
+  uint64_t queue_cap[2] = {}, queue_need[2] = {};
+  uint64_t piece_bytes = 64u << 20, first_piece_bytes = 64u << 20;
+};
+
+struct UploadPlan {
+  std::vector<UploadPiece> pieces;
+  std::vector<UploadStage> stages;
+  uint64_t end[kUploadBufs] = {};
+};
+
+constexpr int kPlanOk = 0;
+constexpr int kPlanInvalid = -22;
+
+inline uint64_t upload_chunks(const UploadShape& s) {
+  if (s.first) return 1 + (s.n - s.first + s.sub - 1) / s.sub;
+  return (s.n + s.sub - 1) / s.sub;
+}
+inline void upload_chunk(const UploadShape& s, uint64_t c, uint64_t* base, uint64_t* cnt) {
+  const uint64_t b = s.first ? (c == 0 ? 0 : s.first + (c - 1) * s.sub) : c * s.sub;
+  const uint64_t cap = s.first && c == 0 ? s.first : s.sub;
+  *base = b;
+  *cnt = std::min(cap, s.n - b);
+}
+
+inline int plan_upload(const UploadShape& s, const uint64_t* roff, const uint32_t* len, UploadPlan* out) {
+  out->pieces.clear();
+  out->stages.clear();
+  for (uint32_t b = 0; b < kUploadBufs; ++b) out->end[b] = s.from[b];
+  const bool bytes_mode = s.mode != kUploadSig;
+  if (s.mode > kUploadBlob || s.n == 0 || s.n > 0xffffffc0ull || s.sub == 0 || s.piece_bytes == 0 ||
+      s.first_piece_bytes == 0)
+    return kPlanInvalid;
+  if (s.n > s.sub && (s.sub % 64) != 0) return kPlanInvalid;
+  if (s.first && (s.mode != kUploadSig || s.first % 64 != 0 || s.first >= s.sub || s.first >= s.n))
+    return kPlanInvalid;
+  if (bytes_mode && (!roff || !len)) return kPlanInvalid;
+  if (s.hash_launches != 1 && !(s.hash_launches == 2 && s.n > s.sub)) return kPlanInvalid;
+  if (s.r_rows > s.n) return kPlanInvalid;
+  for (int i = 0; i < 3; ++i)
+    if (s.out_need[i] > s.out_cap[i]) return kPlanInvalid;
+  if (s.scratch_row && (s.scratch_row > UINT64_MAX / s.n || s.scratch_row * s.n > s.scratch_cap)) return kPlanInvalid;
+  if (s.r_rows && s.r_rows * s.rdec_row > s.rdec_cap) return kPlanInvalid;
+  if (s.key_domain &&
+      (s.n > s.key_max_rows || s.key_off > s.ws_cap || s.key_bytes > s.ws_cap - s.key_off))
+    return kPlanInvalid;
+  for (int j = 0; j < 2; ++j)
+    if (s.queue_need[j] > s.queue_cap[j]) return kPlanInvalid;
+
+  std::vector<uint64_t> ends[kUploadBufs];
+  std::vector<int32_t> idx[kUploadBufs];
+  bool bad = false;
+  auto want = [&](uint32_t b, uint64_t hi) -> int32_t {
+    if (hi > s.cap[b] || s.from[b] > s.cap[b]) {
+      bad = true;
+      return -1;
+    }
+    if (hi <= s.from[b]) return -1;
+    uint64_t at = out->end[b];
+    while (at < hi) {
+      const uint64_t lim = out->pieces.empty() ? std::min(s.first_piece_bytes, s.piece_bytes) : s.piece_bytes;
+      const uint64_t k = std::min(lim, hi - at);
+      out->pieces.push_back(UploadPiece{b, at, k});
+      at += k;
+      ends[b].push_back(at);
+      idx[b].push_back((int32_t)out->pieces.size() - 1);
+    }
+    out->end[b] = at;
+    const size_t p = (size_t)(std::lower_bound(ends[b].begin(), ends[b].end(), hi) - ends[b].begin());
+    return p < idx[b].size() ? idx[b][p] : -1;
+  };
+  auto rows_end = [&](uint64_t a, uint64_t b) {
+    uint64_t e = 0;
+    for (uint64_t i = a; i < b; ++i) {
+      if (roff[i] > UINT64_MAX - len[i]) {
+        bad = true;
+        return (uint64_t)0;
+      }
+      e = std::max(e, roff[i] + len[i]);
+    }
+    return e;
+  };
+  auto stage = [&](uint32_t kind, uint64_t row0, uint64_t rows, std::initializer_list<int32_t> need) {
+    int32_t last = -1;
+    for (int32_t p : need) last = std::max(last, p);
+    out->stages.push_back(UploadStage{kind, row0, rows, last});
+  };
+  auto rows_stage = [&](uint64_t a, uint64_t b) {
+    stage(kStageRows, a, b - a, {want(kBufOff, 8 * s.n), want(kBufLen, 4 * s.n), want(kBufBytes, rows_end(a, b))});
+  };
+  auto verify_stage = [&](uint64_t base, uint64_t cnt) {
+    const uint64_t hi = base + cnt;
+    if (s.mode == kUploadBlob)
+      stage(kStageVerify, base, cnt, {});
+    else if (s.mode == kUploadPre)
+      stage(kStageVerify, base, cnt, {want(kBufSig, 64 * hi), want(kBufPk, 32 * hi)});
+    else
+      stage(kStageVerify, base, cnt, {want(kBufSig, 64 * hi), want(kBufMsg, 32 * hi), want(kBufPk, 32 * hi)});
+  };
+
+  if (s.mode == kUploadPre && s.points_ahead) verify_stage(0, s.n);
+  if (bytes_mode) {
+    const uint64_t h0 = s.hash_launches == 2 ? s.sub : s.n;
+    rows_stage(0, h0);
+    if (h0 < s.n) rows_stage(h0, s.n);
+  }
+  if (s.keys_stage) {
+    if (s.mode == kUploadBlob) stage(kStageKeys, 0, s.n, {});
+    else stage(kStageKeys, 0, s.n, {want(kBufPk, 32 * s.n)});
+  }
+  if (s.r_rows) {
+    if (s.mode == kUploadBlob) stage(kStageR, 0, s.r_rows, {});
+    else stage(kStageR, 0, s.r_rows, {want(kBufSig, 64 * s.r_rows), want(kBufPk, 32 * s.r_rows)});
+  }
+  if (!(s.mode == kUploadPre && s.points_ahead)) {
+    const uint64_t nc = upload_chunks(s);
+    for (uint64_t c = 0; c < nc; ++c) {
+      uint64_t base, cnt;
+      upload_chunk(s, c, &base, &cnt);
+      verify_stage(base, cnt);
+    }
+  }
+  if (bad) {
+    out->pieces.clear();
+    out->stages.clear();
+    for (uint64_t& e : out->end) e = 0;
+    return kPlanInvalid;
+  }
+  return kPlanOk;
+}
+
+}
```
